# vxlerian/cpu-raymarcher

Measured on AMD Instinct MI355X. Metric: frames/sec, 3840x2160 Dense-Grid sphere-trace (+ avg SDF-calls/pixel), higher is better.
Workload: dtype f64

## Files before the change

### cpu_raymarcher_amd/_native.py

```python
import ctypes as C
import os
import subprocess

_PKG = os.path.dirname(os.path.abspath(__file__))
LIB_PATH = os.environ.get("RM_HIP_LIB") or os.path.join(_PKG, "librm_hip.so")
CSRC = os.path.join(_PKG, "csrc")

RM_OK = 0
RM_E_INVALID = -1
RM_E_UNSUPPORTED = -2
RM_E_NO_DEVICE = -3
RM_E_HIP = -4
RM_E_NO_SCENE = -5
RM_E_NOMEM = -6
RM_SCENE_UPLOADED = -(2 ** 31)

_STATUS_NAMES = {0: "RM_OK", -1: "RM_E_INVALID", -2: "RM_E_UNSUPPORTED", -3: "RM_E_NO_DEVICE",
                 -4: "RM_E_HIP", -5: "RM_E_NO_SCENE", -6: "RM_E_NOMEM"}


class RmError(RuntimeError):
    def __init__(self, code, msg):
        super().__init__("%s (%d): %s" % (_STATUS_NAMES.get(code, "?"), code, msg))
        self.code = code
# ... 137 lines not shown
    "rm_last_kernel": (C.c_char_p, [_VP]),
    "rm_version": (C.c_char_p, []),
    "rm_algorithm_from_string": (C.c_int, [C.c_char_p]),
    "rm_accel_from_string": (C.c_int, [C.c_char_p]),
    "rm_shader_from_string": (C.c_int, [C.c_char_p]),
    "rm_preset_count": (C.c_int, []),
    "rm_scene_from_preset": (C.c_int, [_VP, C.c_int32, C.c_int32]),
    "rm_scene_from_spheres": (C.c_int, [_VP, _VP, _VP, C.c_int32, C.c_int32]),
    "rm_scene_edit_spheres": (C.c_int, [_VP, C.POINTER(rm_sphere_edit), C.c_int32]),
    "rm_debug_scene_table": (C.c_int, [_VP, C.c_char_p, C.c_int32, _VP, C.c_int64, C.POINTER(C.c_int64)]),
    "rm_selftest_hypot64": (C.c_int, [_VP, _VP, C.c_int64, C.c_int32, _VP]),
    "rm_scene_from_prims": (C.c_int, [_VP, C.POINTER(rm_prim), C.c_int32, C.c_int32]),
    "rm_make_transform": (C.c_int, [C.c_double, C.c_double, C.c_double, _VP, _VP]),
    "rm_scene_from_nodes": (C.c_int, [_VP, C.POINTER(rm_node), C.c_int32, _VP, C.c_int32, C.c_int32]),
    "rm_scale_transform": (C.c_int, [_VP, C.c_double, C.c_double, C.c_double]),
    "rm_scene_set_time": (C.c_int, [_VP, C.c_double]),
    "rm_selftest_jsmath": (C.c_int, [_VP, C.c_int32, _VP, _VP, C.c_int64, _VP]),
    "rm_scene_get_info": (C.c_int, [_VP, C.POINTER(rm_scene_info)]),
    "rm_camera_from_angles": (C.c_int, [C.c_double, C.c_double, _VP, _VP]),
    "rm_scene_distance": (C.c_int, [_VP, _VP, C.c_int64, _VP, _VP]),
    "rm_debug_wave_distance": (C.c_int, [_VP, _VP, C.c_int64, _VP, _VP]),
    "rm_scene_field": (C.c_int, [_VP, C.POINTER(rm_lattice), _VP, _VP, _VP]),
    "rm_scene_field_device": (C.c_int, [_VP, C.POINTER(rm_lattice), _VP, _VP, _VP, _VP]),
    "rm_lattice_points": (C.c_int, [C.POINTER(rm_lattice), C.c_int64, C.c_int64, _VP]),
    "rm_shade_field_device": (C.c_int, [_VP, C.POINTER(rm_field_shade), C.c_int64, _VP, _VP, _VP]),
    "rm_shade_field": (C.c_int, [_VP, C.POINTER(rm_field_shade), C.c_int64, _VP, _VP]),
    "rm_mesh_field_device": (C.c_int, [_VP, C.POINTER(rm_lattice), _VP, C.c_int32, C.c_double, _VP, C.c_int64, _VP, C.c_int64, _VP, _VP]),
    "rm_scene_mesh": (C.c_int, [_VP, C.POINTER(rm_lattice), C.c_double, _VP, C.c_int64, _VP, C.c_int64, C.POINTER(rm_mesh_info)]),
    "rm_ray_march": (C.c_int, [_VP, C.POINTER(rm_ray_query), C.c_int64, _VP, _VP, _VP, _VP, _VP, _VP]),
    "rm_ray_march_device": (C.c_int, [_VP, C.POINTER(rm_ray_query), C.c_int64, _VP, _VP, _VP, _VP, _VP, _VP, _VP]),
    "rm_camera_rays": (C.c_int, [C.c_int32, C.c_int32, C.c_double, C.c_double, C.c_int32, C.c_int32, _VP, _VP]),
    "rm_ray_pick": (C.c_int, [_VP, C.POINTER(rm_ray_query), C.c_int64, _VP, _VP, _VP, _VP, _VP, _VP, _VP]),
    "rm_ray_pick_device": (C.c_int, [_VP, C.POINTER(rm_ray_query), C.c_int64, _VP, _VP, _VP, _VP, _VP, _VP, _VP, _VP]),
    "rm_ray_light": (C.c_int, [_VP, C.POINTER(rm_ray_query), C.POINTER(rm_light), C.c_int64, _VP, _VP, _VP, _VP, _VP, _VP, _VP, _VP, _VP,
                               _VP]),
    "rm_ray_light_device": (C.c_int, [_VP, C.POINTER(rm_ray_query), C.POINTER(rm_light), C.c_int64, _VP, _VP, _VP, _VP, _VP, _VP, _VP, _VP,
                                      _VP, _VP, _VP]),
    "rm_ray_walk": (C.c_int, [_VP, C.POINTER(rm_ray_query), C.c_int64, _VP, _VP, C.c_int32, _VP, _VP]),
    "rm_ray_walk_device": (C.c_int, [_VP, C.POINTER(rm_ray_query), C.c_int64, _VP, _VP, C.c_int32, _VP, _VP, _VP]),
    "rm_phong_light": (C.c_int, [_VP]),
    "rm_shade_lit_device": (C.c_int, [_VP, C.c_int32, C.c_int32, C.c_int32, _VP, _VP, _VP, _VP, _VP, _VP]),
    "rm_shade_lit": (C.c_int, [_VP, C.c_int32, C.c_int32, C.c_int32, _VP, _VP, _VP, _VP, _VP]),
    "rm_scene_object": (C.c_int, [_VP, C.c_int32, C.POINTER(rm_node), C.c_int32, C.POINTER(C.c_int32)]),
    "rm_render_tile": (C.c_int, [_VP, C.POINTER(rm_job), _VP, _VP, _VP, _VP]),
    "rm_render_tile_device": (C.c_int, [_VP, C.POINTER(rm_job), C.c_int32, _VP, _VP, _VP, _VP, _VP, _VP]),
    "rm_render_frames_device": (C.c_int, [_VP, C.POINTER(rm_job), C.c_int32, _VP, C.c_int32, _VP, _VP, _VP, _VP, _VP, _VP, _VP]),
    "rm_compare_frames_device": (C.c_int, [_VP, C.c_int32, C.c_int32, C.c_int32, C.POINTER(rm_frame_set), C.POINTER(rm_frame_set),
                                           C.c_int32, C.c_int32, _VP, _VP, _VP]),
    "rm_compare_frames": (C.c_int, [_VP, C.c_int32, C.c_int32, C.c_int32, C.POINTER(rm_frame_set), C.POINTER(rm_frame_set),
                                    C.c_int32, C.c_int32, _VP, _VP]),
    "rm_counter_hist_device": (C.c_int, [_VP, C.c_int32, C.c_int32, C.c_int32, _VP, _VP, _VP, C.c_int32, C.c_int32, C.c_int32, C.c_int32,
                                         _VP, _VP]),
    "rm_counter_hist": (C.c_int, [_VP, C.c_int32, C.c_int32, C.c_int32, _VP, _VP, _VP, C.c_int32, C.c_int32, C.c_int32, C.c_int32, _VP]),
    "rm_shade_ranged_device": (C.c_int, [_VP, C.c_int32, C.c_int32, C.c_int32, C.c_int32, _VP, _VP, C.c_uint32, C.c_uint32, _VP, _VP]),
    "rm_shade_ranged": (C.c_int, [_VP, C.c_int32, C.c_int32, C.c_int32, C.c_int32, _VP, _VP, C.c_uint32, C.c_uint32, _VP]),
    "rm_sweep_views": (C.c_int, [C.c_double, C.c_double, C.c_double, C.c_double, C.c_double, C.c_double, C.c_int32, _VP]),
    "rm_render_stripes_device": (C.c_int, [_VP, C.POINTER(rm_job), C.c_int32, C.c_int32, C.c_int32, C.c_int32,
                                           _VP, _VP, _VP, _VP, _VP, _VP]),
    "rm_stripe_rows": (C.c_int, [C.c_int32, C.c_int32, C.c_int32, C.c_int32, C.c_int32]),
    "rm_deal_stripes": (C.c_int, [C.c_int32, C.c_int32, C.c_int32, _VP, _VP]),
    "rm_render_stripe_list_device": (C.c_int, [_VP, C.POINTER(rm_job), C.c_int32, C.c_int32, _VP, C.c_int32,
                                               _VP, _VP, _VP, _VP, _VP, _VP]),
    "rm_assemble_frame_device": (C.c_int, [_VP, _VP, C.c_int64, C.c_int64, C.c_int32, C.c_int32, C.c_int32, _VP,
                                           C.c_int32, C.c_int32, _VP, C.c_int64, _VP, _VP]),
    "rm_shade": (C.c_int, [_VP, C.c_int32, C.c_int32, C.c_int32, _VP, _VP, _VP, _VP, _VP]),
    "rm_shade_device": (C.c_int, [_VP, C.c_int32, C.c_int32, C.c_int32, _VP, _VP, _VP, _VP, _VP, _VP]),
    "rm_reduce_counters": (C.c_int, [_VP, _VP, _VP, C.c_int64, C.POINTER(rm_diagnostics)]),
    "rm_reduce_counters_device": (C.c_int, [_VP, _VP, _VP, C.c_int64, C.POINTER(rm_diagnostics), _VP]),
    "rm_reduce_counters_enqueue": (C.c_int, [_VP, _VP, _VP, C.c_int64, _VP, _VP]),
    "rm_render_attach_diagnostics": (C.c_int, [_VP, _VP]),
    "rm_partition_rows": (C.c_int, [C.c_int32, C.c_int32, C.c_int32, C.POINTER(C.c_int32), C.POINTER(C.c_int32)]),
    "rm_selftest_hypot": (C.c_int, [_VP, _VP, C.c_int64, _VP]),
    "rm_selftest_fastdiv": (C.c_int, [_VP, C.c_uint64, C.c_int64, C.POINTER(C.c_uint64)]),
    "rm_selftest_recip": (C.c_int, [_VP, C.c_int, _VP]),
    "rm_debug_read_stamps": (C.c_int, [_VP, _VP]),
    "rm_debug_read_wave_times": (C.c_int, [_VP, _VP]),
    "rm_debug_read_batch_log": (C.c_int, [_VP, _VP]),
    "rm_debug_read_counts": (C.c_int, [_VP, _VP]),
    "rm_debug_read_lpt_costs": (C.c_int, [_VP, _VP, C.c_int64]),
    "rm_debug_launch_fill": (C.c_int, [_VP, C.c_int32, C.POINTER(C.c_int32)]),
    "rm_debug_last_launch": (C.c_int, [_VP, C.POINTER(C.c_uint32)]),
    "rm_debug_overlap_fill": (C.c_int, [_VP, C.c_int32, C.c_int64, C.POINTER(C.c_int32)]),
    "rm_debug_step_box": (C.c_int, [_VP, C.POINTER(C.c_int32)]),
    "rm_rtc_source": (C.c_int, [_VP, C.c_char_p, C.c_int64, C.POINTER(C.c_int64)]),
    "rm_rtc_compile_check": (C.c_int, [_VP, C.c_int32, C.c_int32, C.c_char_p, C.c_int64, C.POINTER(C.c_double)]),
    "rm_rtc_status": (C.c_int, [_VP, C.POINTER(C.c_int32), C.POINTER(C.c_int32), C.c_char_p, C.c_int64]),
    "rm_set_option": (C.c_int, [_VP, C.c_char_p, C.c_int64]),
    "rm_get_option": (C.c_int, [_VP, C.c_char_p, C.POINTER(C.c_int64)]),
}

_lib = None


def build(force=False, verbose=False):
    srcs = [os.path.join(CSRC, f) for f in os.listdir(CSRC) if f.endswith((".hip", ".cpp", ".h"))]
    srcs.append(os.path.join(os.path.dirname(_PKG), "include", "rm_raymarch.h"))
    if not force and os.path.exists(LIB_PATH) and all(
            os.path.getmtime(LIB_PATH) >= os.path.getmtime(s) for s in srcs):
        return LIB_PATH
    cmd = ["make", "-j%d" % min(8, os.cpu_count() or 1), "-C", CSRC, "all"] + (["-B"] if force else [])
    subprocess.check_call(cmd, stdout=None if verbose else subprocess.DEVNULL)
    return LIB_PATH


def lib():
    global _lib
    if _lib is None:
        if not os.path.exists(LIB_PATH):
            raise ImportError(
                "cpu_raymarcher_amd: %s is missing. Build it with `python -c 'import __graft_entry__ as g; "
                "g.build()'` or `make -C cpu_raymarcher_amd/csrc`. There is no CPU fallback." % LIB_PATH)
        try:
            import torch
        except ImportError:
            pass
        L = C.CDLL(LIB_PATH)
        for name, (res, args) in SIGNATURES.items():
            if os.environ.get("RM_HIP_LIB") and not hasattr(L, name):
                continue
            fn = getattr(L, name)
            fn.restype = res
            fn.argtypes = args
        _lib = L
    return _lib


def check(ctx, rc):
    if rc == RM_OK:
        return
    msg = lib().rm_last_error(ctx).decode() if ctx else ""
    raise (RmUnsupported if rc == RM_E_UNSUPPORTED else RmError)(rc, msg)
```

### cpu_raymarcher_amd/context.py

```python
import ctypes as C

import numpy as np

from . import _native as N


def _is_torch(x):
    return type(x).__module__.startswith("torch")


def _ptr(x):
    if x is None:
        return None
    if _is_torch(x):
        return C.c_void_p(x.data_ptr())
    return x.ctypes.data_as(C.c_void_p)


_BPP = {"depth": 1, "normal": 3, "sdf": 2, "iters": 2, "rgba": 4}


def _check_buffers(npx, bufs, need_device=None):
    on_dev = None
    for name, b in bufs.items():
# ... 50 lines not shown
    if not (_is_torch(hist) or isinstance(hist, np.ndarray)):
        raise ValueError("hist must be a numpy array or a torch tensor")
    d = bool(_is_torch(hist) and hist.is_cuda)
    contiguous = hist.is_contiguous() if _is_torch(hist) else hist.flags["C_CONTIGUOUS"]
    nbytes = hist.numel() * hist.element_size() if _is_torch(hist) else hist.nbytes
    if not contiguous or nbytes < 2128 * max(0, n_frames):
        raise ValueError("hist must be a contiguous buffer of 2128 bytes per frame")
    if on_dev is not None and on_dev != d:
        raise ValueError("buffers must be all on the host or all on the device")
    return d


def percentile(record, permille):
    p = int(permille)
    if not 0 <= p <= 1000:
        raise ValueError("permille must be in [0, 1000]")
    M = int(record["pixels"])
    if M == 0:
        return 0, 0
    r = p * (M - 1) // 1000
    b = int(np.searchsorted(np.cumsum(np.asarray(record["bins"], dtype=np.uint64)), r, side="right"))
    shift, mn, mx = int(record["shift"]), int(record["min"]), int(record["max"])
    return max(mn, b << shift), (mx if b == 255 else min(mx, ((b + 1) << shift) - 1))


def _current_stream_ptr():
    import torch
    return C.c_void_p(torch.cuda.current_stream().cuda_stream)


class Context:

    def __init__(self, device=0):
        self._h = C.c_void_p()
        self.device = -1 if device is None else int(device)
        rc = N.lib().rm_create(self.device, C.byref(self._h))
        if rc != N.RM_OK:
            raise N.RmError(rc, "rm_create(device=%d) failed: no usable HIP device" % self.device)

    def close(self):
        if self._h:
            N.lib().rm_destroy(self._h)
            self._h = C.c_void_p()

    def __del__(self):
        try:
            self.close()
        except Exception:
            pass

    def __enter__(self):
        return self

    def __exit__(self, *a):
        self.close()

    def set_option(self, key, value):
        N.check(self._h, N.lib().rm_set_option(self._h, key.encode(), int(value)))

    def get_option(self, key):
        v = C.c_int64(0)
        N.check(self._h, N.lib().rm_get_option(self._h, key.encode(), C.byref(v)))
        return v.value

    def launch_fill(self, asked):
        v = C.c_int32(0)
        N.check(self._h, N.lib().rm_debug_launch_fill(self._h, int(asked), C.byref(v)))
        return v.value

    def last_launch(self):
        out = (C.c_uint32 * 4)()
        N.check(self._h, N.lib().rm_debug_last_launch(self._h, out))
        return dict(workgroups=out[0], threads=out[1], lds_bytes=out[2], cus=out[3])

    def overlap_fill(self, asked, items):
        v = C.c_int32(0)
        N.check(self._h, N.lib().rm_debug_overlap_fill(self._h, int(asked), int(items), C.byref(v)))
        return v.value

    def step_box(self):
        out = (C.c_int32 * 6)()
        N.check(self._h, N.lib().rm_debug_step_box(self._h, out))
        return dict(last=bool(out[0]), planned=bool(out[1]), reason=out[2], list_cap=out[3], list_cap_without=out[4], table_bytes=out[5])

    def scene_from_preset(self, index, accel):
        N.check(self._h, N.lib().rm_scene_from_preset(self._h, int(index), int(accel)))

    def scene_from_spheres(self, centers, radii, accel):
        c = np.ascontiguousarray(centers, dtype=np.float32).reshape(-1, 3)
        r = np.ascontiguousarray(radii, dtype=np.float64).reshape(-1)
        if len(c) != len(r):
            raise ValueError("centers and radii differ in length")
        N.check(self._h, N.lib().rm_scene_from_spheres(self._h, _ptr(c), _ptr(r), len(r), int(accel)))

    def scene_from_prims(self, prims, accel):
        prims = list(prims)
        arr = (N.rm_prim * max(1, len(prims)))()
        for i, (t, m, par) in enumerate(prims):
            arr[i].type = int(t)
            for k in range(16):
                arr[i].world_to_local[k] = float(m[k])
            for k in range(3):
                arr[i].params[k] = float(par[k]) if k < len(par) else 0.0
        N.check(self._h, N.lib().rm_scene_from_prims(self._h, arr, len(prims), int(accel)))

    def scene_from_nodes(self, nodes, roots, accel):
        nodes = list(nodes)
        arr = (N.rm_node * max(1, len(nodes)))()
        for i, (t, a, b, m, par) in enumerate(nodes):
            arr[i].type, arr[i].child_a, arr[i].child_b = int(t), int(a), int(b)
            for k in range(16):
                arr[i].world_to_local[k] = 0.0 if m is None else float(m[k])
            for k in range(6):
                arr[i].params[k] = float(par[k]) if k < len(par) else 0.0
        r = np.ascontiguousarray(roots, dtype=np.int32)
        N.check(self._h, N.lib().rm_scene_from_nodes(self._h, arr, len(nodes), _ptr(r), len(r), int(accel)))

    def edit_spheres(self, edits):
        if isinstance(edits, C.Array) and edits._type_ is N.rm_sphere_edit:
            arr, n = edits, len(edits)
        else:
            edits = list(edits)
            n = len(edits)
            arr = (N.rm_sphere_edit * max(1, n))()
            for k, e in enumerate(edits):
                arr[k].op = N.EDIT_OPS[e[0]] if isinstance(e[0], str) else int(e[0])
                arr[k].index = int(e[1])
                if len(e) > 2:
                    arr[k].center[:] = [float(v) for v in np.asarray(e[2], np.float32).reshape(3)]
                    arr[k].radius = float(e[3])
        N.check(self._h, N.lib().rm_scene_edit_spheres(self._h, arr, n))

    def scene_table(self, name, from_device=True):
        size = C.c_int64(0)
        key = name.encode()
        N.check(self._h, N.lib().rm_debug_scene_table(self._h, key, int(bool(from_device)), None, 0, C.byref(size)))
        out = np.zeros(size.value, np.uint8)
        N.check(self._h, N.lib().rm_debug_scene_table(self._h, key, int(bool(from_device)), _ptr(out), out.size, C.byref(size)))
        return out.view(N.SCENE_TABLES.get(name, "u1"))

    def selftest_hypot64(self, xyz, on_device=True):
        a = np.ascontiguousarray(xyz, dtype=np.float64).reshape(-1, 3)
        out = np.zeros(len(a), np.float64)
        N.check(self._h, N.lib().rm_selftest_hypot64(self._h, _ptr(a), len(a), int(bool(on_device)), _ptr(out)))
        return out

    def scene_set_time(self, time):
        N.check(self._h, N.lib().rm_scene_set_time(self._h, float(time)))

    def selftest_jsmath(self, fn, a, b=None):
        a = np.ascontiguousarray(a, dtype=np.float64)
        b = None if b is None else np.ascontiguousarray(b, dtype=np.float64)
        out = np.zeros_like(a)
        N.check(self._h, N.lib().rm_selftest_jsmath(self._h, int(fn), _ptr(a), _ptr(b), a.size, _ptr(out)))
        return out

    def scene_info(self):
        info = N.rm_scene_info()
        N.check(self._h, N.lib().rm_scene_get_info(self._h, C.byref(info)))
        d = {k: getattr(info, k) for k, _ in info._fields_ if k not in ("root_min", "root_max", "reserved")}
        d["root_min"] = [float(v) for v in info.root_min]
        d["root_max"] = [float(v) for v in info.root_max]
        d["prog_slots"], d["prog_vals"], d["prog_instructions"] = info.program & 0xFF, (info.program >> 8) & 0xFF, info.program >> 16
        return d

    def scene_distance(self, points):
# ... 710 lines not shown
```

### cpu_raymarcher_amd/csrc/rm_api.cpp

```cpp
#include <hip/hip_runtime_api.h>

#include <algorithm>
#include <array>
#include <cerrno>
#include <climits>
#include <cmath>
#include <cstdio>
#include <cstdlib>
#include <cstring>
#include <functional>
#include <limits>
#include <map>
#include <unordered_map>
#include <new>
#include <string>
#include <vector>

#include "../../include/rm_raymarch.h"
#include "rm_diag.h"
#include "rm_kernels.h"
#include "rm_rtc.h"
#include "rm_scene_host.h"

namespace {

#define RM_SCENE_ARRAYS(X)                                                                                                        \
    X(spheres, 1) X(radii, 1) X(bvh, 1) X(bvh_prims, 1) X(oct, 1) X(oct_prims, 1) X(pq_cells, 1) X(pq_list, 1) X(nn_cells, 1)      \
    X(nn_list, 1) X(prims, 1) X(prog, 1) X(obj_ranges, 1) X(oct_recs, 1) X(oct_lut, 1) X(oct_sub_hdr, 1) X(oct_sub_list, 1)       \
    X(slot_object, 0) X(ext_cells, 1) X(ext_list, 1) X(step_tab, 1)

struct DeviceScene {
#define RM_X(name, always) decltype(rmh::HostScene::name)::value_type *name = nullptr;
    RM_SCENE_ARRAYS(RM_X)
#undef RM_X
    uint16_t *bvh_leaves = nullptr;
    int32_t bvh_leaf_count = 0;
};

struct SceneDesc {
    enum Kind { kSpheres, kPrims, kNodes } kind = kSpheres;
    std::vector<float> centers;
    std::vector<double> radii;
    std::vector<rmh::PrimDesc> prims;
    std::vector<rmh::NodeDesc> nodes;
    std::vector<int> roots;
};

struct LaunchSlots {
    static constexpr unsigned kLaunches = 1024, kHeads = 64, kHeadWords = 64;
    unsigned int *heads = nullptr;
    RmDiagBlock *blocks = nullptr;
    unsigned int head_slot = 0, block_slot = 0;

    hipError_t init() {
        const size_t head_bytes = sizeof(unsigned int) * kLaunches * kHeads * kHeadWords, block_bytes = sizeof(RmDiagBlock) * kLaunches;
        hipError_t e = hipMalloc(reinterpret_cast<void **>(&heads), head_bytes);
        if (e == hipSuccess) e = hipMemset(heads, 0, head_bytes);
        if (e == hipSuccess) e = hipMalloc(reinterpret_cast<void **>(&blocks), block_bytes);
        return e == hipSuccess ? hipMemset(blocks, 0, block_bytes) : e;
    }
    void release() {
        (void)hipFree(heads);
        (void)hipFree(blocks);
    }
    unsigned int *take_heads() { return heads ? heads + static_cast<size_t>(kHeads) * kHeadWords * (head_slot++ % kLaunches) : nullptr; }
    RmDiagBlock *take_block() { return blocks ? blocks + block_slot++ % kLaunches : nullptr; }
};

struct RingClaims {
    struct Claim {
        size_t first, n;
        hipEvent_t done;
    };
    size_t next = 0;
    std::vector<Claim> claims;

    void retire_all() {
        for (Claim &c : claims) (void)hipEventDestroy(c.done);
        claims.clear();
        next = 0;
    }
    hipError_t take(size_t n, size_t cap, size_t *first) {
        if (next + n > cap) next = 0;
        const size_t lo = next, hi = next + n;
        for (size_t k = 0; k < claims.size();) {
            const Claim c = claims[k];
            if (c.first < hi && lo < c.first + c.n) {
                const hipError_t e = hipEventSynchronize(c.done);
                if (e != hipSuccess) return e;
                (void)hipEventDestroy(c.done);
                claims.erase(claims.begin() + static_cast<std::ptrdiff_t>(k));
            } else ++k;
        }
        *first = lo;
        next = hi;
        return hipSuccess;
    }
    void launched(size_t first, size_t n, hipStream_t stream) {
        hipEvent_t ev = nullptr;
        if (hipEventCreateWithFlags(&ev, hipEventDisableTiming) == hipSuccess && hipEventRecord(ev, stream) == hipSuccess) {
            claims.push_back(Claim{first, n, ev});
            return;
        }
        if (ev) (void)hipEventDestroy(ev);
        (void)hipStreamSynchronize(stream);
    }
};

struct FrameRing {
    static constexpr size_t kFrames = 4096;
    RmFrameView *host = nullptr, *dev = nullptr;
    RmFrameDiagBlock *blocks = nullptr;
    size_t cap = 0;
    RingClaims owners;

    void release() {
        owners.retire_all();
        (void)hipHostFree(host);
        (void)hipFree(dev);
        (void)hipFree(blocks);
        host = dev = nullptr;
        blocks = nullptr;
        cap = 0;
    }
    hipError_t take(size_t n, size_t *first) {
        if (n > cap) {
            hipError_t e = hipDeviceSynchronize();
            if (e != hipSuccess) return e;
            release();
            const size_t want = n > kFrames ? n : kFrames;
            e = hipHostMalloc(reinterpret_cast<void **>(&host), want * sizeof(RmFrameView), hipHostMallocDefault);
            if (e == hipSuccess) e = hipMalloc(reinterpret_cast<void **>(&dev), want * sizeof(RmFrameView));
            if (e == hipSuccess) e = hipMalloc(reinterpret_cast<void **>(&blocks), want * sizeof(RmFrameDiagBlock));
            if (e == hipSuccess) e = hipMemset(blocks, 0, want * sizeof(RmFrameDiagBlock));
            if (e != hipSuccess) {
                release();
                return e;
            }
            cap = want;
        }
        return owners.take(n, cap, first);
    }
    void launched(size_t first, size_t n, hipStream_t stream) { owners.launched(first, n, stream); }
};

struct CompareRing {
    static constexpr size_t kEntries = 4096;
// ... 133 lines not shown
        for (auto &u : t.users) {
            (void)hipEventSynchronize(u.second);
            (void)hipEventDestroy(u.second);
        }
        t.users.clear();
        t.valid = false;
        const size_t n = static_cast<size_t>(oct_nodes);
        if (t.nodes < n) {
            (void)hipFree(t.dev);
            t.dev = nullptr;
            t.nodes = 0;
            if (hipMalloc(reinterpret_cast<void **>(&t.dev), n * sizeof(RmOctFrameNode)) == hipSuccess) t.nodes = n;
            else (void)hipGetLastError();
        }
        if (!t.dev || rm_launch_oct_frame_table(oct, oct_nodes, origin, t.dev, stream) != hipSuccess) return nullptr;
        for (int a = 0; a < 3; ++a) t.origin[a] = origin[a];
        t.gen = gen;
        t.valid = true;
        t.builder = stream;
        if (!t.built && hipEventCreateWithFlags(&t.built, hipEventDisableTiming) != hipSuccess) t.built = nullptr;
        if (!t.built || hipEventRecord(t.built, stream) != hipSuccess) (void)hipStreamSynchronize(stream);
        cur = k;
        return &t;
    }
    static void read_by(Table &t, hipStream_t stream) {
        hipEvent_t ev = nullptr;
        for (auto &u : t.users)
            if (u.first == stream) ev = u.second;
        if (!ev) {
            if (hipEventCreateWithFlags(&ev, hipEventDisableTiming) == hipSuccess) t.users.emplace_back(stream, ev);
            else ev = nullptr;
        }
        if (ev) (void)hipEventRecord(ev, stream);
        else (void)hipStreamSynchronize(stream);
    }
    void release() {
        for (Table &t : slots) {
            (void)hipFree(t.dev);
            for (auto &u : t.users) (void)hipEventDestroy(u.second);
            if (t.built) (void)hipEventDestroy(t.built);
        }
    }
};

}

struct rm_ctx {
    int device = -1;
    bool has_device = false;
    std::string err = "";
    hipStream_t stream = nullptr;

    bool have_scene = false;
    bool scene_is_uploaded = false;
    int scene_preset = 0;
    rmh::HostScene host;
    DeviceScene dev;

    bool have_uploaded = false;
    SceneDesc uploaded;
    double time = 0.0;

    void *scratch = nullptr;
    size_t scratch_bytes = 0;
    hipEvent_t scratch_busy = nullptr;
    RmDiagDevice *d_diag = nullptr;
    float light[3] = {0, 0, 0};

    int64_t opt_tile_w = 8;
    bool tile_w_set = false;
    int64_t opt_filter = 1;
    int64_t opt_lds = 1;
    int64_t opt_kernel = 0;
    int64_t opt_list_cap = 32;
    int64_t opt_coop = 1;
    int64_t opt_grid = 1;
    int64_t opt_nn = 2;
    int64_t opt_ext = 1;
    int64_t opt_blocks_per_cu = 6;
    int64_t opt_lds_fill = 0;
    int64_t opt_min_fill = 1;
    int64_t opt_overlap_fill = 1;
    int hw_queues = 4;
    uint32_t last_v2_shape[4] = {0, 0, 0, 0};
    int64_t opt_item_wide = 0;
    int64_t opt_multi_step = 1;
    int64_t opt_step_box = 1;
    int64_t opt_lds_kb = 0;
    int64_t opt_refill = 64;
    int64_t opt_recs = 1;
    int64_t opt_static = 0;
    int64_t opt_lut = 1;
    int64_t opt_cull = 1;
    int64_t opt_rel = 1;
    int64_t opt_uniform = 1;
    int64_t opt_sub = 1;
    int64_t opt_hw_xcd = 1;
    int64_t opt_v1_lists = 1;
    int64_t opt_v1_block = 64;
    int64_t opt_oct_lean = 1;
    int64_t opt_lpt = 1;
    LaunchSlots slots;
    LptRing lpt;
    OctTableRing oct_tables;
    FrameRing frames;
    CompareRing compare;
    HistRing hists;
    unsigned long long scene_gen = 0;
    int64_t opt_n0_batch = 64;
    int64_t opt_length = 0;
    const char *last_kernel = "";
    std::string last_kernel_kept;
    int64_t opt_device_build = 1;
    int64_t opt_specialise = 1;
    int64_t opt_rtc_spheres = 16;
    int64_t opt_prune = 1;
    std::string rtc_src;
    std::map<int, rmrtc::Kernel> rtc_kernels;
    std::vector<rmrtc::Kernel> rtc_owned;
    std::map<int, std::string> rtc_failed;
    std::string rtc_log;
    struct V2Special {
        int launches = 0;
        int state = 0;
        bool lite = false;
        rmrtc::Kernel k;
    };
    std::unordered_map<uint64_t, V2Special> v2_special;
    int64_t opt_v2_after = 3;
    struct DevTable {
        std::vector<int32_t> host;
        int32_t *dev = nullptr;
    };
    std::vector<DevTable> tables;
    int64_t opt_item_px = 128;
    void *diag_next = nullptr;
    unsigned long long *d_stamps = nullptr;
    int num_cus = 256;
};

namespace {

int fail(rm_ctx *ctx, int code, const std::string &msg) {
    if (ctx) ctx->err = msg;
    return code;
}

int hip_fail(rm_ctx *ctx, hipError_t e, const char *what) {
    return fail(ctx, RM_E_HIP, std::string(what) + ": " + hipGetErrorString(e));
}

int read_hw_queues() {
    const char *s = std::getenv("GPU_MAX_HW_QUEUES");
    if (!s || !*s) return 4;
    char *end = nullptr;
    errno = 0;
    const long long v = std::strtoll(s, &end, 10);
    if (errno || end == s || *end != '\0' || v <= 0) return 4;
    return static_cast<int>(std::min<long long>(v, INT_MAX));
}

int launch_fill(int asked, int queues, bool min_fill) {
    if (!min_fill) return asked;
    const int q = queues > 0 ? queues : 4;
    return std::max(asked, (RM_V2_WAVES + q - 1) / q);
}

int overlap_fill(int asked, int queues, bool min_fill, bool overlap) {
    const int floor = launch_fill(asked, queues, min_fill);
    const int q = queues > 0 ? queues : 4;
    if (!min_fill || !overlap || q >= RM_V2_WAVES) return floor;
    const int per_mille = 436 * q;
    return std::max(floor, std::min(RM_V2_WAVES, (RM_V2_WAVES * 1000 + per_mille - 1) / per_mille));
}

int obtain_kernel(rm_ctx *ctx, const std::string &src, int accel, bool other, bool length_sqrt, rmrtc::Kernel &k) {
    if (ctx->opt_specialise == 2) return rmrtc::compile_async(ctx->device, src, accel, other, length_sqrt, k, ctx->rtc_log);
    bool cached = false;
    if (!rmrtc::compile_cached(ctx->device, src, accel, other, length_sqrt, k, ctx->rtc_log, &cached)) return -1;
    if (!cached) ctx->rtc_owned.push_back(k);
    return 1;
}

const rmrtc::Kernel *specialised_kernel(rm_ctx *ctx, int accel, bool other) {
    if (!ctx->opt_specialise || ctx->rtc_src.empty() || !ctx->has_device) return nullptr;
    const int key = (accel * 2 + (other ? 1 : 0)) * 2 + (ctx->opt_length ? 1 : 0);
    auto it = ctx->rtc_kernels.find(key);
    if (it != ctx->rtc_kernels.end()) return &it->second;
    if (ctx->rtc_failed.count(key)) return nullptr;
    rmrtc::Kernel k;
    const int st = obtain_kernel(ctx, ctx->rtc_src, accel, other, ctx->opt_length != 0, k);
    if (st < 0) ctx->rtc_failed[key] = ctx->rtc_log;
    if (st <= 0) return nullptr;
    return &(ctx->rtc_kernels[key] = k);
}

}

const void *rm_rtc_v2_hook(const RmRenderParams &p, int accel, bool lds, bool ur, bool rel, bool length_sqrt) {
    rm_ctx *ctx = static_cast<rm_ctx *>(p.rtc_ctx);
    if (!ctx || !ctx->opt_specialise || ctx->opt_v2_after <= 0) return nullptr;
    const int bits = (accel & 3) | (lds ? 4 : 0) | (ur ? 8 : 0) | (rel ? 16 : 0) | rmrtc::kV2Bit;
    rm_ctx::V2Special &e = ctx->v2_special[rmrtc::v2_fixed_hash(p, bits | (length_sqrt ? 512 : 0))];
    if (e.state == 1) return e.k.render;
    if (e.state < 0) return nullptr;
    if (e.state == 0 && ++e.launches < ctx->opt_v2_after) return nullptr;
    for (;;) {
        const int st = obtain_kernel(ctx, rmrtc::v2_fixed_source(p, !e.lite), bits, false, length_sqrt, e.k);
        e.state = st > 0 ? 1 : (st < 0 ? -1 : 2);
        if (st >= 0 || e.lite) break;
        e.lite = true;
        e.state = 0;
    }
    return e.state == 1 ? e.k.render : nullptr;
}

namespace {

hipError_t launch_render(rm_ctx *ctx, const RmRenderParams &p_in, RmDiagDevice *diag_out, hipStream_t stream) {
    RmRenderParams p = p_in;
#if !defined(RM_STAMPS) && !defined(RM_COUNTS) && !defined(RM_STAMPS_LOG) && !defined(RM_STAMPS_CLAIM)
    p.rtc_ctx = ctx;
#endif
    const bool empty = p.local_rows <= 0 || p.width <= 0;
    const bool v2 = p.variant == 2 && p.algorithm == 0;
    const bool lean_oct = p.accel == 1 && p.oct_lean && !p.general && p.algorithm == 0 && p.oct_lut && p.oct_recs && p.filter;
    const rmrtc::Kernel *special = v2 || lean_oct ? nullptr : specialised_kernel(ctx, p.accel, p.algorithm != 0);
    p.rtc_function = special ? special->render : nullptr;
    OctTableRing::Table *oct_table = lean_oct ? ctx->oct_tables.acquire(ctx->scene_gen, p.oct, p.oct_nodes, p.origin_d, stream) : nullptr;
    p.oct_frame = oct_table ? oct_table->dev : nullptr;
    if (ctx->opt_lpt && v2) ctx->lpt.acquire(p);
    if (v2 && !empty) p.tile_counters = ctx->slots.take_heads();
    p.diag_out = diag_out;
    RmDiagDevice *reduce_after = nullptr;
    if (p.diag_out && !v2 && !empty && p.sdf && p.iters) {
        reduce_after = p.diag_out;
        p.diag_out = nullptr;
    }
    p.diag_block = !empty && (p.diag_out || v2) ? ctx->slots.take_block() : nullptr;
    if (p.diag_out && empty) {
        const hipError_t ei = rm_launch_reduce_init(p.diag_out, stream);
        if (ei != hipSuccess) return ei;
    }
    hipError_t e = ctx->opt_length ? rm_launch_render_sqrt(p, stream, &ctx->last_kernel, ctx->last_v2_shape)
                                   : rm_launch_render(p, stream, &ctx->last_kernel, ctx->last_v2_shape);
    if (special && !empty) ctx->last_kernel = special->name.c_str();
    if (e == hipSuccess && reduce_after) {
        e = rm_launch_reduce_init(reduce_after, stream);
        if (e == hipSuccess) e = rm_launch_reduce(p.sdf, p.iters, static_cast<int64_t>(p.local_rows) * p.width, reduce_after, stream);
    }
    if (oct_table) OctTableRing::read_by(*oct_table, stream);
    if (e == hipSuccess && p.lpt_perm_out) ctx->lpt.launched(stream);
    return e;
}

#define RM_HIP(ctx, call)                                       \
    do {                                                        \
        hipError_t e_ = (call);                                 \
        if (e_ != hipSuccess) return hip_fail(ctx, e_, #call); \
    } while (0)

#define RM_NEED_DEVICE(ctx, text)                                             \
    do {                                                                      \
        if (!(ctx)) return RM_E_INVALID;                                      \
        if (!(ctx)->has_device) return fail(ctx, RM_E_NO_DEVICE, text);       \
    } while (0)

void free_device_scene(rm_ctx *ctx) {
    for (auto &k : ctx->rtc_owned) rmrtc::release(k);
    ctx->rtc_owned.clear();
    ctx->rtc_kernels.clear();
    ctx->v2_special.clear();
    ctx->rtc_failed.clear();
    ctx->last_kernel = "";
    if (!ctx->has_device) return;
    DeviceScene &d = ctx->dev;
#define RM_X(name, always) (void)hipFree(d.name);
    RM_SCENE_ARRAYS(RM_X)
#undef RM_X
    (void)hipFree(d.bvh_leaves);
    d = DeviceScene();
}

int device_table(rm_ctx *ctx, const int32_t *host, size_t n, const int32_t **out) {
    for (auto &t : ctx->tables)
        if (t.host.size() == n && std::memcmp(t.host.data(), host, n * sizeof(int32_t)) == 0) {
            *out = t.dev;
            return RM_OK;
        }
    if (ctx->tables.size() >= 256) {
        RM_HIP(ctx, hipDeviceSynchronize());
        for (auto &t : ctx->tables) (void)hipFree(t.dev);
        ctx->tables.clear();
    }
    rm_ctx::DevTable t;
    t.host.assign(host, host + n);
    RM_HIP(ctx, hipMalloc(reinterpret_cast<void **>(&t.dev), (n ? n : 1) * sizeof(int32_t)));
    if (n) RM_HIP(ctx, hipMemcpy(t.dev, host, n * sizeof(int32_t), hipMemcpyHostToDevice));
    *out = t.dev;
    ctx->tables.push_back(std::move(t));
    return RM_OK;
}

template <typename T>
int upload_vec(rm_ctx *ctx, const std::vector<T> &v, T **out) {
    *out = nullptr;
    const size_t bytes = (v.empty() ? 1 : v.size()) * sizeof(T);
    RM_HIP(ctx, hipMalloc(reinterpret_cast<void **>(out), bytes));
    if (!v.empty()) RM_HIP(ctx, hipMemcpy(*out, v.data(), v.size() * sizeof(T), hipMemcpyHostToDevice));
    return RM_OK;
}

std::vector<uint16_t> cull_leaf_table(const std::vector<RmBvhNode> &bvh) {
    std::vector<uint16_t> leaves;
    bool ok = !bvh.empty() && bvh.size() < 65536;
    std::vector<int> parent(bvh.size(), -1);
    for (size_t i = 0; ok && i < bvh.size(); ++i) {
        if (bvh[i].leaf >= 0) continue;
        for (size_t c = i + 1; c < static_cast<size_t>(bvh[i].skip) && c < bvh.size(); c = static_cast<size_t>(bvh[c].skip)) {
            parent[c] = static_cast<int>(i);
            if (bvh[c].skip <= static_cast<int>(c)) { ok = false; break; }
        }
    }
    for (size_t i = 0; ok && i < bvh.size(); ++i) {
        if (parent[i] >= 0)
            for (int k = 0; k < 3; ++k)
                if (!(bvh[i].lo[k] >= bvh[parent[i]].lo[k] && bvh[i].hi[k] <= bvh[parent[i]].hi[k])) ok = false;
        for (int k = 0; k < 3; ++k)
            if (!(bvh[i].lo[k] <= bvh[i].hi[k])) ok = false;
        if (i > 0 && parent[i] < 0) ok = false;
        if (bvh[i].leaf >= 0 && (bvh[i].leaf & 0xFF) > 0) leaves.push_back(static_cast<uint16_t>(i));
    }
    if (!ok || leaves.size() > 256) leaves.clear();
    return leaves;
}

int upload_scene(rm_ctx *ctx) {
    ctx->rtc_src.clear();
    if (ctx->host.program) {
        ctx->rtc_src = rmrtc::scene_source(ctx->host.prog, ctx->host.obj_ranges, ctx->host.prog_tree, ctx->host.prog_roots, ctx->opt_prune != 0, ctx->host.bvh,
                                           ctx->host.bvh_prims, false);
    } else if (ctx->host.general ? ctx->host.prims.size() <= 32 : static_cast<int64_t>(ctx->host.spheres.size()) < ctx->opt_rtc_spheres) {
        std::vector<RmInstr> prog;
        std::vector<int32_t> ranges, roots;
        std::vector<rmh::ProgTreeNode> tree;
        if (rmh::leaf_objects(ctx->host, prog, ranges, tree, roots))
            ctx->rtc_src = rmrtc::scene_source(prog, ranges, tree, roots, false, ctx->host.bvh, ctx->host.bvh_prims, true);
    }
    if (!ctx->has_device) {
        free_device_scene(ctx);
        return RM_OK;
    }
    RM_HIP(ctx, hipSetDevice(ctx->device));
    RM_HIP(ctx, hipDeviceSynchronize());
    free_device_scene(ctx);
    ctx->scene_gen++;
    int rc;
#define RM_X(name, always) \
    if ((always || !ctx->host.name.empty()) && (rc = upload_vec(ctx, ctx->host.name, &ctx->dev.name))) return rc;
    RM_SCENE_ARRAYS(RM_X)
#undef RM_X
    const std::vector<uint16_t> leaves = cull_leaf_table(ctx->host.bvh);
    ctx->dev.bvh_leaf_count = static_cast<int32_t>(leaves.size());
    return upload_vec(ctx, leaves, &ctx->dev.bvh_leaves);
}

int clamp_preset(int idx) { return idx < 0 ? 0 : (idx > rmh::kPresetCount - 1 ? rmh::kPresetCount - 1 : idx); }
int norm_accel(int a) { return (a == RM_ACCEL_OCTREE || a == RM_ACCEL_BVH) ? a : RM_ACCEL_NONE; }

int set_scene(rm_ctx *ctx, const SceneDesc &d, int accel, bool uploaded, int preset, const rmh::PairLoops *loops = nullptr) {
    std::string err;
    rmh::HostScene hs;
    rmh::set_length_mode(static_cast<int>(ctx->opt_length));
    bool ok = false;
    switch (d.kind) {
        case SceneDesc::kSpheres: ok = rmh::build_scene(hs, d.centers.data(), d.radii.data(), static_cast<int>(d.radii.size()), accel, err, loops); break;
        case SceneDesc::kPrims: ok = rmh::build_scene_general(hs, d.prims.data(), static_cast<int>(d.prims.size()), accel, err); break;
        case SceneDesc::kNodes:
            ok = rmh::build_scene_nodes(hs, d.nodes.data(), static_cast<int>(d.nodes.size()), d.roots.data(), static_cast<int>(d.roots.size()), accel, err);
            break;
    }
    if (!ok) {
        const bool unsupported = err.find("BVH leaf") != std::string::npos || (d.kind == SceneDesc::kNodes && err.find("RM_PROG_MAX") != std::string::npos);
        return fail(ctx, unsupported ? RM_E_UNSUPPORTED : RM_E_INVALID, err);
    }
    hs.preset = preset;
    ctx->host = std::move(hs);
    ctx->have_scene = true;
    ctx->scene_is_uploaded = uploaded;
    ctx->scene_preset = preset;
    return upload_scene(ctx);
}

int set_uploaded_scene(rm_ctx *ctx, SceneDesc &&d, int32_t accel) {
    const int rc = set_scene(ctx, d, norm_accel(accel), true, RM_SCENE_UPLOADED);
    if (rc) return rc;
    ctx->uploaded = std::move(d);
    ctx->have_uploaded = true;
    return RM_OK;
}

bool preset_desc(int preset, SceneDesc &d) {
    d.kind = SceneDesc::kSpheres;
    if (rmh::preset_spheres(preset, d.centers, d.radii)) return true;
    d.kind = SceneDesc::kPrims;
    if (rmh::preset_prims(preset, d.prims)) return true;
    d.kind = SceneDesc::kNodes;
    return rmh::preset_nodes(preset, d.nodes, d.roots);
}


struct DevMem {
    void *p = nullptr;
    DevMem() = default;
    DevMem(const DevMem &) = delete;
    DevMem &operator=(const DevMem &) = delete;
    ~DevMem() {
        if (p) (void)hipFree(p);
    }
    hipError_t alloc(size_t bytes) { return hipMalloc(&p, bytes ? bytes : 1); }
    template <typename T>
    hipError_t put(const T *src, size_t n, hipStream_t stream) {
        hipError_t e = alloc(n * sizeof(T));
        if (e == hipSuccess && n) e = hipMemcpyAsync(p, src, n * sizeof(T), hipMemcpyHostToDevice, stream);
        return e;
    }
    template <typename T>
    T *as() const { return static_cast<T *>(p); }
};

#define RM_TRY(call)                            \
    do {                                        \
        if ((call) != hipSuccess) return false; \
    } while (0)

template <typename E>
bool device_cand_lists(rm_ctx *ctx, const rmh::HostScene &s, const std::vector<int32_t> *ids, const std::vector<RmCandGrid> &grids,
                       int cells_per_grid, double u0, bool use_root, bool cap255, const std::vector<uint32_t> *order,
                       std::vector<uint32_t> &hdr, std::vector<E> &list) {
    const size_t n = s.spheres.size(), n_cells = grids.size() * static_cast<size_t>(cells_per_grid);
    if (!n || !n_cells || n != s.radii.size() || n > 0x7FFFFFFFu || (order && order->size() != n_cells)) return false;
    RM_TRY(hipSetDevice(ctx->device));
    hipStream_t st = ctx->stream;
    std::vector<double> sp(4 * n);
    for (size_t i = 0; i < n; ++i) {
        sp[4 * i] = s.spheres[i].cx;
        sp[4 * i + 1] = s.spheres[i].cy;
// ... 177 lines not shown
        for (const RmInstr &ins : ctx->host.prog)
            if (ins.op == 3) p.general = 3;
    }
    p.prims = ctx->dev.prims;
    p.prog = ctx->dev.prog;
    p.obj_ranges = ctx->dev.obj_ranges;
    p.prog_slots = ctx->host.prog_slots;
    p.prog_vals = ctx->host.prog_vals;
    p.accel = ctx->host.accel;
    p.bvh_nodes = static_cast<int32_t>(ctx->host.bvh.size());
    p.oct_nodes = static_cast<int32_t>(ctx->host.oct.size());
    p.spheres = ctx->dev.spheres;
    p.radii = ctx->dev.radii;
    p.bvh = ctx->dev.bvh;
    p.bvh_prims = ctx->dev.bvh_prims;
    p.oct = ctx->dev.oct;
    p.oct_prims = ctx->dev.oct_prims;
    p.oct_lut = ctx->opt_lut ? ctx->dev.oct_lut : nullptr;
    p.ext_cells = ctx->dev.ext_cells;
    p.ext_list = ctx->dev.ext_list;
    for (int k = 0; k < 3; ++k) {
        p.ext_dim[k] = ctx->host.ext_dim[k];
        p.ext_origin[k] = ctx->host.ext_origin[k];
        p.ext_inv[k] = ctx->host.ext_inv[k];
    }
    p.use_ext = (ctx->opt_ext && ctx->host.accel == RM_ACCEL_BVH && !ctx->host.ext_cells.empty() && ctx->host.ext_dim[0] > 0) ? 1 : 0;
}


int ensure_scene(rm_ctx *ctx, int32_t preset_index, int32_t accel_in) {
    const int accel = norm_accel(accel_in);
    if (preset_index == RM_SCENE_UPLOADED) {
        if (!ctx->have_uploaded) return fail(ctx, RM_E_NO_SCENE, "no scene uploaded with rm_scene_from_spheres");
        if (ctx->have_scene && ctx->scene_is_uploaded && ctx->host.accel == accel) return RM_OK;
        return set_scene(ctx, ctx->uploaded, accel, true, RM_SCENE_UPLOADED);
    }
    const int preset = clamp_preset(preset_index);
    if (ctx->have_scene && !ctx->scene_is_uploaded && ctx->scene_preset == preset && ctx->host.accel == accel)
        return RM_OK;
    SceneDesc d;
    if (preset_desc(preset, d)) return set_scene(ctx, d, accel, false, preset);
    return fail(ctx, RM_E_UNSUPPORTED, "scene preset " + std::to_string(preset) + " is not on the native path");
}

size_t align_up(size_t v, size_t a) { return (v + a - 1) / a * a; }

struct Staging {
    rm_ctx *ctx;
    size_t total = 0;
    size_t region(size_t bytes) {
        const size_t offset = total;
        total += align_up(bytes, 256);
        return offset;
    }
    int reserve() const { return reserve_for(ctx->stream); }
    int reserve_for(hipStream_t user) const {
        if (ctx->scratch_busy) RM_HIP(ctx, hipStreamWaitEvent(user, ctx->scratch_busy, 0));
        const size_t bytes = total ? total : 256;
        if (bytes <= ctx->scratch_bytes) return RM_OK;
        if (ctx->scratch) {
            RM_HIP(ctx, hipDeviceSynchronize());
            (void)hipFree(ctx->scratch);
            ctx->scratch = nullptr;
            ctx->scratch_bytes = 0;
        }
        RM_HIP(ctx, hipMalloc(&ctx->scratch, bytes));
        ctx->scratch_bytes = bytes;
        return RM_OK;
    }
    template <typename T>
    T *at(size_t offset) const { return reinterpret_cast<T *>(static_cast<char *>(ctx->scratch) + offset); }
    hipError_t in(size_t offset, const void *host, size_t bytes) const { return hipMemcpyAsync(at<char>(offset), host, bytes, hipMemcpyHostToDevice, ctx->stream); }
    hipError_t zero(size_t offset, size_t bytes) const { return hipMemsetAsync(at<char>(offset), 0, bytes, ctx->stream); }
    hipError_t out(void *host, size_t offset, size_t bytes) const { return hipMemcpyAsync(host, at<char>(offset), bytes, hipMemcpyDeviceToHost, ctx->stream); }
    hipError_t sync() const { return hipStreamSynchronize(ctx->stream); }
    hipError_t keep(hipStream_t user) const {
        if (!ctx->scratch_busy) {
            const hipError_t e = hipEventCreateWithFlags(&ctx->scratch_busy, hipEventDisableTiming);
            if (e != hipSuccess) return e;
        }
        return hipEventRecord(ctx->scratch_busy, user);
    }
};

int fill_params(rm_ctx *ctx, const rm_job *job, RmRenderParams &p) {
    if (!job) return fail(ctx, RM_E_INVALID, "null job");
    if (job->height <= 0 || job->width < 0) return fail(ctx, RM_E_INVALID, "width must be >= 0 and height > 0");
    if (!std::isfinite(job->camera_pitch) || !std::isfinite(job->camera_yaw))
        return fail(ctx, RM_E_INVALID, "non-finite camera angle");
    if (job->algorithm < RM_ALG_SPHERE_TRACER || job->algorithm > RM_ALG_ADAPTIVE_STEP_V3)
        return fail(ctx, RM_E_INVALID, "unknown algorithm enum (use rm_algorithm_from_string)");
    int rc = ensure_scene(ctx, job->scene_preset_index, job->acceleration_structure);
    if (rc) return rc;
    std::memset(&p, 0, sizeof p);
    p.width = job->width;
    p.height = job->height;
    p.y_start = job->y_start;
    p.y_end = job->y_end;
    p.algorithm = job->algorithm;
    p.overshoot = std::isnan(job->overshoot_factor) ? 1.2 : job->overshoot_factor;
    p.step_size = std::isnan(job->step_size) ? 0.1 : job->step_size;
    p.local_rows = job->y_end > job->y_start ? job->y_end - job->y_start : 0;
    p.stripe_rows = 0;
    p.n_parts = 1;
    p.part = 0;
    rmh::camera_from_angles(job->camera_pitch, job->camera_yaw, p.rot, p.origin);
    std::memcpy(p.light, ctx->light, sizeof p.light);
    for (int k = 0; k < 9; ++k) p.rot_d[k] = p.rot[k];
    for (int k = 0; k < 3; ++k) {
        p.origin_d[k] = p.origin[k];
        p.light_d[k] = p.light[k];
    }
    fill_scene_view(ctx, p);
    if (!std::isfinite(job->time)) return fail(ctx, RM_E_INVALID, "non-finite time");
    ctx->time = job->time;
    p.time = job->time;
    p.tile_w = static_cast<int32_t>(ctx->opt_tile_w);
    p.nodes_in_lds = static_cast<int32_t>(ctx->opt_lds);
    p.filter = static_cast<int32_t>(ctx->opt_filter);
    p.variant = static_cast<int32_t>(ctx->opt_kernel);
    if (p.variant == 0)
        p.variant = (ctx->host.accel == RM_ACCEL_OCTREE || ctx->host.spheres.size() < 8 ||
                     (ctx->opt_specialise && !ctx->rtc_src.empty() && rmrtc::available(nullptr) &&
                      static_cast<int64_t>(ctx->host.spheres.size()) < ctx->opt_rtc_spheres))
                        ? 1
                        : 2;
    if (p.algorithm != RM_ALG_SPHERE_TRACER) p.variant = 1;
    if (ctx->host.general) p.variant = 1;
    if (p.variant == 1 && !ctx->tile_w_set) p.tile_w = 8;
    p.list_cap = static_cast<int32_t>(ctx->opt_list_cap);
    p.coop = static_cast<int32_t>(ctx->opt_coop);
    p.bvh_prim_count = static_cast<int32_t>(ctx->host.bvh_prims.size());
    p.oct_prim_count = static_cast<int32_t>(ctx->host.oct_prims.size());
    p.blocks_per_cu = static_cast<int32_t>(ctx->opt_blocks_per_cu);
    p.launch_per_cu = launch_fill(p.blocks_per_cu, ctx->hw_queues, ctx->opt_min_fill != 0);
    p.overlap_per_cu = overlap_fill(p.blocks_per_cu, ctx->hw_queues, ctx->opt_min_fill != 0, ctx->opt_overlap_fill != 0);
    p.num_cus = ctx->num_cus;
    p.refill_threshold = static_cast<int32_t>(ctx->opt_refill);
    p.hw_xcd = static_cast<int32_t>(ctx->opt_hw_xcd);
    p.item_px = static_cast<int32_t>(ctx->opt_item_px);
    p.stamps = ctx->d_stamps;
    for (int k = 0; k < 3; ++k) {
        p.pq_dim[k] = ctx->host.pq_dim[k];
        p.pq_origin[k] = ctx->host.pq_origin[k];
        p.pq_inv[k] = ctx->host.pq_inv[k];
        p.pq_cell[k] = ctx->host.pq_inv[k] > 0.f ? static_cast<float>((1.0 / static_cast<double>(ctx->host.pq_inv[k])) * 0.9999) : 0.f;
    }
    p.pq_cell_count = static_cast<int32_t>(ctx->host.pq_cells.size());
    p.pq_list_count = static_cast<int32_t>(ctx->host.pq_list.size());
    p.use_grid = (ctx->opt_grid && !ctx->host.pq_cells.empty()) ? 1 : 0;
    p.pq_cells = ctx->dev.pq_cells;
    p.pq_list = ctx->dev.pq_list;
    p.bvh_leaves = ctx->dev.bvh_leaves;
    p.bvh_leaf_count = (ctx->opt_cull && ctx->host.accel == RM_ACCEL_BVH) ? ctx->dev.bvh_leaf_count : 0;
    p.nn_cells = ctx->dev.nn_cells;
    p.nn_list = ctx->dev.nn_list;
    p.nn_cell_count = static_cast<int32_t>(ctx->host.nn_cells.size());
    p.nn_list_count = static_cast<int32_t>(ctx->host.nn_list.size());
    const bool nn_on = ctx->opt_nn == 1 || (ctx->opt_nn == 2 && ctx->host.spheres.size() <= 512);
    p.use_nn = (p.use_grid && nn_on && !ctx->host.nn_cells.empty()) ? 1 : 0;
    p.leaf_order = ctx->host.leaf_order ? 1 : 0;
    p.rel_boxes = static_cast<int32_t>(ctx->opt_rel);
    p.n0_batch = static_cast<int32_t>(ctx->opt_n0_batch);
    p.v1_lists = static_cast<int32_t>(ctx->opt_v1_lists);
    p.v1_block = static_cast<int32_t>(ctx->opt_v1_block);
    p.oct_lean = static_cast<int32_t>(ctx->opt_oct_lean);
    p.v1_list_offset = -1;
    p.prim_filter = (ctx->opt_filter && ctx->host.general && !ctx->host.program && ctx->host.prim_filter_ok &&
                     ctx->host.spheres.size() == ctx->host.prims.size()) ? 1 : 0;
    p.lds_budget_kb = static_cast<int32_t>(ctx->opt_lds_kb);
    p.lds_fill = static_cast<int32_t>(ctx->opt_lds_fill);
    p.item_wide = static_cast<int32_t>(ctx->opt_item_wide);
    p.multi_step = static_cast<int32_t>(ctx->opt_multi_step);
    p.step_tab = ctx->dev.step_tab;
    p.sb_bins = ctx->host.sb_bins;
    p.sb_stride = ctx->host.sb_stride;
    for (int k = 0; k < 3; ++k) {
        p.sb_origin[k] = ctx->host.sb_origin[k];
        p.sb_inv[k] = ctx->host.sb_inv[k];
    }
    p.step_box = (ctx->opt_step_box && ctx->opt_multi_step && ctx->host.accel == RM_ACCEL_BVH && !ctx->host.step_tab.empty() &&
                  (ctx->dev.step_tab || !ctx->has_device)) ? 1 : 0;
    p.uniform_radius = 0;
    if (ctx->opt_uniform && !ctx->host.general && ctx->host.spheres.size() >= 2 &&
        ctx->host.spheres.size() <= 256) {
        const auto &sp = ctx->host.spheres;
        const auto &rd = ctx->host.radii;
        bool same = rd.size() == sp.size();
        for (size_t k = 1; same && k < sp.size(); ++k)
            same = std::memcmp(&sp[k].rf, &sp[0].rf, sizeof(float)) == 0 && std::memcmp(&rd[k], &rd[0], sizeof(double)) == 0;
        p.uniform_radius = same ? 1 : 0;
    }
    for (int k = 0; k < 3; ++k) {
        p.nn_dim[k] = ctx->host.nn_dim[k];
        p.nn_inv[k] = ctx->host.nn_inv[k];
    }
    p.oct_recs = ctx->opt_recs ? ctx->dev.oct_recs : nullptr;
    p.oct_sub_hdr = (ctx->opt_sub && ctx->opt_recs) ? ctx->dev.oct_sub_hdr : nullptr;
    p.oct_sub_list = ctx->dev.oct_sub_list;
    return RM_OK;
}

template <typename Launch>
int read_mismatches(rm_ctx *ctx, Launch launch, uint64_t *mismatches) {
    RM_HIP(ctx, hipSetDevice(ctx->device));
    Staging st{ctx};
    const size_t o = st.region(sizeof(unsigned long long));
    const int rc = st.reserve();
    if (rc) return rc;
    RM_HIP(ctx, st.zero(o, sizeof(unsigned long long)));
    RM_HIP(ctx, launch(st.at<unsigned long long>(o)));
    unsigned long long h = 0;
    RM_HIP(ctx, st.out(&h, o, sizeof h));
    RM_HIP(ctx, st.sync());
    *mismatches = h;
    return RM_OK;
}

int norm_shader(int s) { return (s >= RM_SHADE_NORMAL && s <= RM_SHADE_ITERATION_HEATMAP) ? s : RM_SHADE_NORMAL; }

int fill_query_params(rm_ctx *ctx, const rm_ray_query *q, RmRenderParams &p) {
    const double scene_time = ctx->time;
    rm_job job;
    std::memset(&job, 0, sizeof job);
    job.width = 1;
    job.height = 1;
    job.y_end = 1;
    job.time = q->time;
    const bool known = q->algorithm >= RM_ALG_SPHERE_TRACER && q->algorithm <= RM_ALG_ADAPTIVE_STEP_V3;
    job.algorithm = known ? q->algorithm : RM_ALG_SPHERE_TRACER;
    job.scene_preset_index = ctx->scene_is_uploaded ? RM_SCENE_UPLOADED : ctx->scene_preset;
    job.acceleration_structure = ctx->host.accel;
    job.overshoot_factor = q->overshoot_factor;
    job.step_size = q->step_size;
    const int rc = fill_params(ctx, &job, p);
    ctx->time = scene_time;
    p.rtc_function = nullptr;
// ... 1680 lines not shown
    const bool ok = rmrtc::compile(ctx->rtc_src, norm_accel(accel), other != 0, ctx->opt_length != 0, false, k, text);
    if (seconds) *seconds = k.compile_seconds;
    copy_text(text, log, cap, nullptr);
    if (ok) return RM_OK;
    if (text.compare(0, 8, "refused:") == 0) return fail(ctx, RM_E_UNSUPPORTED, "hiprtc: the specialised kernel spills and would not be loaded (see the log)");
    return fail(ctx, RM_E_INVALID, "hiprtc: the specialised kernel did not compile (see the log)");
}

int rm_rtc_status(rm_ctx *ctx, int32_t *compiled, int32_t *failed, char *log, int64_t cap) {
    if (!ctx) return RM_E_INVALID;
    int v2_ready = 0, v2_failed = 0;
    for (const auto &kv : ctx->v2_special) {
        v2_ready += kv.second.state == 1;
        v2_failed += kv.second.state < 0;
    }
    if (compiled) *compiled = static_cast<int32_t>(ctx->rtc_kernels.size()) + v2_ready;
    if (failed) *failed = static_cast<int32_t>(ctx->rtc_failed.size()) + v2_failed;
    std::string why;
    if (!rmrtc::available(&why)) return copy_text(why, log, cap, nullptr);
    return copy_text(ctx->rtc_log, log, cap, nullptr);
}

int rm_debug_read_lpt_costs(rm_ctx *ctx, uint8_t *out, int64_t n) {
    if (!out) return RM_E_INVALID;
    RM_NEED_DEVICE(ctx, "host-only context");
    const uint8_t *costs = ctx->lpt.last_costs();
    if (!costs || n < 0 || static_cast<size_t>(n) > LptRing::kPerSlot) return fail(ctx, RM_E_INVALID, "no costs recorded");
    RM_HIP(ctx, hipSetDevice(ctx->device));
    RM_HIP(ctx, hipDeviceSynchronize());
    RM_HIP(ctx, hipMemcpy(out, costs, static_cast<size_t>(n), hipMemcpyDeviceToHost));
    return RM_OK;
}

int rm_debug_launch_fill(rm_ctx *ctx, int32_t asked, int32_t *effective) {
    if (!ctx || !effective) return RM_E_INVALID;
    if (asked < 1 || asked > 8) return fail(ctx, RM_E_INVALID, "blocks_per_cu must be in [1, 8]");
    *effective = launch_fill(asked, ctx->hw_queues, ctx->opt_min_fill != 0);
    return RM_OK;
}

int rm_debug_overlap_fill(rm_ctx *ctx, int32_t asked, int64_t items, int32_t *effective) {
    if (!ctx || !effective) return RM_E_INVALID;
    if (asked < 1 || asked > 8) return fail(ctx, RM_E_INVALID, "blocks_per_cu must be in [1, 8]");
    if (items < 0) return fail(ctx, RM_E_INVALID, "items must not be negative");
    const bool min_fill = ctx->opt_min_fill != 0;
    *effective = rm_v2_overlap_per_cu(launch_fill(asked, ctx->hw_queues, min_fill),
                                      overlap_fill(asked, ctx->hw_queues, min_fill, ctx->opt_overlap_fill != 0), items, ctx->num_cus);
    return RM_OK;
}

int rm_debug_last_launch(rm_ctx *ctx, uint32_t out[4]) {
    if (!ctx || !out) return RM_E_INVALID;
    for (int k = 0; k < 3; ++k) out[k] = ctx->last_v2_shape[k];
    out[3] = static_cast<uint32_t>(ctx->num_cus);
    return RM_OK;
}

int rm_debug_step_box(rm_ctx *ctx, int32_t out[6]) {
    if (!ctx || !out) return RM_E_INVALID;
    for (int k = 0; k < 6; ++k) out[k] = 0;
    out[0] = static_cast<int32_t>(ctx->last_v2_shape[3]);
    if (!ctx->have_scene) return fail(ctx, RM_E_NO_SCENE, "no scene set");
    rm_job job;
    std::memset(&job, 0, sizeof job);
    job.width = job.height = job.y_end = 64;
    job.algorithm = RM_ALG_SPHERE_TRACER;
    job.scene_preset_index = ctx->scene_is_uploaded ? RM_SCENE_UPLOADED : ctx->scene_preset;
    job.acceleration_structure = ctx->host.accel;
    job.overshoot_factor = job.step_size = std::nan("");
    const double scene_time = ctx->time;
    RmRenderParams p;
    const int rc = fill_params(ctx, &job, p);
    ctx->time = scene_time;
    if (rc) return rc;
    out[5] = static_cast<int32_t>(ctx->host.step_tab.size() * sizeof(uint32_t));
    RmRenderParams plain = p;
    plain.step_box = 0;
    out[4] = rm_v2_plan(plain).list_cap;
    const RmV2Plan plan = rm_v2_plan(p);
    out[3] = plan.list_cap;
    const bool v2 = p.variant == 2 && p.algorithm == 0 && p.accel == 2;
    out[1] = v2 && plan.step_box ? 1 : 0;
    out[2] = out[1] ? 0 : (ctx->host.step_tab.empty() && v2 && ctx->opt_step_box && ctx->opt_multi_step ? 2 : (v2 && plan.refused ? 3 : 1));
    return RM_OK;
}

enum OptionKind {
    kSwitch,
    kRange,
    kZeroOrRange,
    kSet,
};
struct OptionRow {
    const char *key;
    int64_t rm_ctx::*member;
    OptionKind kind;
    int64_t v[4];
    const char *error;
};
static const OptionRow kOptions[] = {
    {"tile_w", &rm_ctx::opt_tile_w, kSet, {8, 16, 32, 64}, "tile_w must be 8, 16, 32 or 64"},
    {"filter", &rm_ctx::opt_filter, kSwitch, {}, nullptr},
    {"nodes_in_lds", &rm_ctx::opt_lds, kSwitch, {}, nullptr},
    {"kernel", &rm_ctx::opt_kernel, kRange, {0, 2}, "kernel must be 0 (auto), 1 or 2"},
    {"list_cap", &rm_ctx::opt_list_cap, kRange, {1, 64}, "list_cap must be in [1, 64]"},
    {"coop", &rm_ctx::opt_coop, kSwitch, {}, nullptr},
    {"recs", &rm_ctx::opt_recs, kSwitch, {}, nullptr},
    {"lut", &rm_ctx::opt_lut, kSwitch, {}, nullptr},
    {"uniform", &rm_ctx::opt_uniform, kSwitch, {}, nullptr},
    {"lds_kb", &rm_ctx::opt_lds_kb, kZeroOrRange, {16, 64}, "lds_kb must be 0 (auto) or in [16, 64]"},
    {"multi_step", &rm_ctx::opt_multi_step, kSwitch, {}, nullptr},
    {"step_box", &rm_ctx::opt_step_box, kSwitch, {}, nullptr},
    {"item_wide", &rm_ctx::opt_item_wide, kSwitch, {}, nullptr},
    {"prune", &rm_ctx::opt_prune, kSwitch, {}, nullptr},
    {"rtc_spheres", &rm_ctx::opt_rtc_spheres, kRange, {0, 33}, "rtc_spheres must be 0..33"},
    {"specialise_v2_after", &rm_ctx::opt_v2_after, kRange, {0, 1000000}, "specialise_v2_after must be 0 (never) .. 1000000 launches"},
    {"specialise", &rm_ctx::opt_specialise, kRange, {0, 2}, "specialise must be 0, 1 or 2"},
    {"lds_fill", &rm_ctx::opt_lds_fill, kSwitch, {}, nullptr},
    {"min_fill", &rm_ctx::opt_min_fill, kSwitch, {}, nullptr},
    {"overlap_fill", &rm_ctx::opt_overlap_fill, kSwitch, {}, nullptr},
    {"cull", &rm_ctx::opt_cull, kSwitch, {}, nullptr},
    {"rel", &rm_ctx::opt_rel, kSwitch, {}, nullptr},
    {"static", &rm_ctx::opt_static, kRange, {0, 95}, "static must be in [0, 95] percent"},
    {"sub", &rm_ctx::opt_sub, kSwitch, {}, nullptr},
    {"refill", &rm_ctx::opt_refill, kRange, {1, 64}, "refill must be in [1, 64]"},
    {"item_px", &rm_ctx::opt_item_px, kSet, {64, 128, 256, 256}, "item_px must be 64, 128 or 256"},
    {"hw_xcd", &rm_ctx::opt_hw_xcd, kSwitch, {}, nullptr},
    {"grid", &rm_ctx::opt_grid, kSwitch, {}, nullptr},
    {"nn", &rm_ctx::opt_nn, kRange, {0, 2}, "nn must be 0 (off), 1 (on) or 2 (auto)"},
    {"ext", &rm_ctx::opt_ext, kSwitch, {}, nullptr},
    {"blocks_per_cu", &rm_ctx::opt_blocks_per_cu, kRange, {1, 8}, "blocks_per_cu must be in [1, 8]"},
    {"v1_lists", &rm_ctx::opt_v1_lists, kSwitch, {}, nullptr},
    {"v1_block", &rm_ctx::opt_v1_block, kSet, {64, 128, 256, 256}, "v1_block must be 64, 128 or 256"},
    {"oct_lean", &rm_ctx::opt_oct_lean, kSwitch, {}, nullptr},
    {"lpt", &rm_ctx::opt_lpt, kSwitch, {}, nullptr},
    {"n0_batch", &rm_ctx::opt_n0_batch, kRange, {1, 64}, "n0_batch must be in [1, 64]"},
    {"device_build", &rm_ctx::opt_device_build, kSwitch, {}, nullptr},
    {"length", &rm_ctx::opt_length, kRange, {0, 1}, "length must be 0 (Math.hypot) or 1 (Math.sqrt)"},
};

static const OptionRow *find_option(const char *key) {
    for (const OptionRow &o : kOptions)
        if (!std::strcmp(key, o.key)) return &o;
    return nullptr;
}

int rm_set_option(rm_ctx *ctx, const char *key, int64_t value) {
    if (!ctx || !key) return RM_E_INVALID;
    const OptionRow *o = find_option(key);
    if (!o) return fail(ctx, RM_E_INVALID, std::string("unknown option ") + key);
    bool ok = true;
    switch (o->kind) {
        case kSwitch: value = value ? 1 : 0; break;
        case kRange: ok = value >= o->v[0] && value <= o->v[1]; break;
        case kZeroOrRange: ok = value == 0 || (value >= o->v[0] && value <= o->v[1]); break;
        case kSet: ok = std::find(std::begin(o->v), std::end(o->v), value) != std::end(o->v); break;
    }
    if (!ok) return fail(ctx, RM_E_INVALID, o->error);
    const bool changed = ctx->*(o->member) != value;
    ctx->*(o->member) = value;
    if (o->member == &rm_ctx::opt_tile_w) ctx->tile_w_set = true;
    if (o->member == &rm_ctx::opt_length && changed && ctx->have_scene) {
        ctx->have_scene = false;
        return ensure_scene(ctx, ctx->scene_is_uploaded ? RM_SCENE_UPLOADED : ctx->scene_preset, ctx->host.accel);
    }
    return RM_OK;
}

int rm_get_option(const rm_ctx *ctx, const char *key, int64_t *value) {
    if (!ctx || !key || !value) return RM_E_INVALID;
    const OptionRow *o = find_option(key);
    if (!o) return RM_E_INVALID;
    *value = ctx->*(o->member);
    return RM_OK;
}

}
```

### cpu_raymarcher_amd/csrc/rm_kernels.h

```cpp
#pragma once
#ifndef __HIPCC_RTC__
#include <hip/hip_runtime_api.h>
#include <stdint.h>
#endif

#include "rm_types.h"

struct RmDiagDevice {
    unsigned long long total_sdf;
    unsigned long long total_iters;
    unsigned int max_sdf;
    unsigned int min_sdf;
    unsigned long long pad;
};

#ifdef RM_LENGTH_SQRT
#define RM_LEN_VARIANT(name) name##_sqrt
#define RM_LEN_TAG " [length=sqrt]"
#define RM_LEN_IS_SQRT true
#else
#define RM_LEN_VARIANT(name) name
#define RM_LEN_TAG ""
#define RM_LEN_IS_SQRT false
#endif

enum { RM_CMP_NONE = -1, RM_CMP_SDF = 0, RM_CMP_ITERS = 1, RM_CMP_DEPTH = 2, RM_CMP_NORMAL = 3, RM_CMP_SURFACE = 4 };
struct RmCompareStats {
    unsigned long long pixels;
    unsigned long long sums[14];
    unsigned int max_abs_depth, max_abs_normal;
};
struct RmComparePartial {
    unsigned long long v[16];
};
struct RmCompareArgs {
    const uint8_t *depth_a, *depth_b, *normal_a, *normal_b;
    const uint16_t *sdf_a, *sdf_b, *iters_a, *iters_b;
    uint8_t *rgba;
    RmCompareStats *stats;
    RmComparePartial *partials;
    unsigned int *counters;
    long long npx;
    unsigned int gain;
};

constexpr int RM_HIST_NBINS = 256;
struct RmCounterHist {
    unsigned long long pixels, sum;
    unsigned int min, max, range_lo, range_hi, shift, reserved;
    unsigned int bins[RM_HIST_NBINS];
};
struct RmFrameHist {
    RmCounterHist sdf, iters;
};
struct RmHistScratch {
    unsigned int bins[2][RM_HIST_NBINS];
    unsigned long long sum[2];
    unsigned int max[2], inv_min[2];
    unsigned int ticket, pad[3];
};
struct RmHistArgs {
    const uint16_t *sdf, *iters;
    const uint8_t *normal;
    RmFrameHist *hist;
    RmHistScratch *scratch;
    long long npx;
    unsigned int shift, lo_permille, hi_permille;
    unsigned int want_surface;
};
struct RmShadeRangedArgs {
    const uint16_t *values;
    const RmFrameHist *hist;
    uint8_t *rgba;
    long long npx;
    unsigned int counter, lo, hi;
};
struct RmShadeLitArgs {
    const uint8_t *depth, *normal;
    const float *lit, *ao;
    uint8_t *rgba;
    long long npx;
    double light[3];
};
struct RmRays {
    const float *origins, *dirs;
    long long n;
};
struct RmQueryArgs {
    int32_t want_normal, pad;
    const int32_t *slot_obj;
    double *t;
    uint32_t *iters, *sdf;
    float *normal;
    int32_t *object;
};
struct RmLightArgs {
    const float *origins, *dirs;
    double *t;
    uint32_t *iters, *sdf;
    float *normal;
    float *lit, *ao;
    uint32_t *iters2, *sdf2;
    long long n;
    double bias, ao_step, ao_strength;
    float light[3];
    int ao_samples;
};
// ... 16 lines not shown
};
struct RmFieldArgs {
    double origin[3], du[3], dv[3], dw[3];
    double *dist;
    float *dist32;
    uint32_t *count;
    long long first, n;
    long long block_first;
    unsigned int nu, nv;
};
struct RmShadeFieldArgs {
    const void *values;
    uint8_t *rgba;
    long long n;
    double range, band, line;
    unsigned int lo, hi;
    int map, pad;
};
#define RM_MESH_BLOCK 256
#define RM_MESH_SCAN_STEP 1024
struct RmMeshInfo {
    long long n_vertices, n_quads, n_holes, reserved;
};
struct RmMeshArgs {
    double origin[3], du[3], dv[3], dw[3];
    const void *values;
    double iso;
    float *vertices;
    uint32_t *quads;
    RmMeshInfo *info;
    uint32_t *map;
    uint32_t *totals;
    long long n, cap_vertices, cap_quads;
    unsigned int nu, nv, nw, n_blocks;
    int f32, pad;
};
struct RmCandGrid {
    double org[3], w[3];
    int32_t dim[3];
    int32_t first, n, pad;
};
#define RM_CAND_NO_LIST 0xFFFFFFFFu
struct RmCandArgs {
    const RmCandGrid *grids;
    const double *spheres;
    const int32_t *ids;
    uint32_t *counts;
    double *u;
    const uint32_t *offsets;
    long long n_cells;
    unsigned long long list_len;
    double u0;
    double root_lo[3], root_hi[3];
    int32_t n_grids, cells_per_grid, n_spheres, n_ids, use_root, pad;
};
struct RmEmptyDistArgs {
    const float *boxes, *prim_lo, *prim_hi;
    double *out;
    int32_t n_nodes, n_prims;
};

#ifndef __HIPCC_RTC__
hipError_t rm_launch_cand_count(const RmCandArgs &a, hipStream_t stream);
hipError_t rm_launch_cand_fill(const RmCandArgs &a, void *list, int elem_bytes, hipStream_t stream);
hipError_t rm_launch_empty_dist(const RmEmptyDistArgs &a, hipStream_t stream);
hipError_t rm_launch_hypot64(const double *xyz, int64_t n, double *out, hipStream_t stream);

hipError_t rm_launch_render(const RmRenderParams &p, hipStream_t stream, const char **kernel_name, uint32_t *v2_shape = nullptr);
hipError_t rm_launch_render_sqrt(const RmRenderParams &p, hipStream_t stream, const char **kernel_name, uint32_t *v2_shape = nullptr);

const void *rm_rtc_v2_hook(const RmRenderParams &p, int accel, bool lds, bool ur, bool rel, bool length_sqrt);

hipError_t rm_launch_render_v2(const RmRenderParams &p, hipStream_t stream, const char **kernel_name, uint32_t *shape = nullptr);
hipError_t rm_launch_render_v2_sqrt(const RmRenderParams &p, hipStream_t stream, const char **kernel_name, uint32_t *shape = nullptr);

#define RM_V2_OVERLAP_ITEMS_PER_WAVE 3
inline int rm_v2_overlap_per_cu(int floor_per_cu, int candidate, long long items, int cus) {
    if (candidate <= floor_per_cu || cus <= 0) return floor_per_cu;
    const long long needed = (items + 3) / 4, resident = static_cast<long long>(cus) * candidate;
    const long long waves = 4 * (needed < resident ? needed : resident);
    return items >= RM_V2_OVERLAP_ITEMS_PER_WAVE * waves ? candidate : floor_per_cu;
}

struct RmV2Plan {
    bool lds, rel;
    int list_cap, step_box, tier, refused;
    size_t scene_bytes, list_bytes;
};
RmV2Plan rm_v2_plan(const RmRenderParams &p);

hipError_t rm_launch_wave_distance(const RmRenderParams &p, const float *points, int64_t n, double *dist, uint32_t *count, hipStream_t stream);
hipError_t rm_launch_wave_distance_sqrt(const RmRenderParams &p, const float *points, int64_t n, double *dist, uint32_t *count, hipStream_t stream);

hipError_t rm_launch_oct_frame_table(const RmOctNode *nodes, int n, const double origin[3], RmOctFrameNode *out, hipStream_t stream);

hipError_t rm_launch_shade(int shader, int64_t n, const uint8_t *depth, const uint8_t *normal,
                           const uint16_t *sdf, const uint16_t *iters, uint8_t *rgba,
                           const float light[3], hipStream_t stream);

hipError_t rm_launch_reduce_init(RmDiagDevice *acc, hipStream_t stream);

hipError_t rm_launch_reduce(const uint16_t *sdf, const uint16_t *iters, int64_t n, RmDiagDevice *acc,
                            hipStream_t stream);

hipError_t rm_launch_distance(const RmRenderParams &p, const float *points, int64_t n, double *dist,
                              uint32_t *count, hipStream_t stream);
hipError_t rm_launch_distance_sqrt(const RmRenderParams &p, const float *points, int64_t n, double *dist,
                                   uint32_t *count, hipStream_t stream);

hipError_t rm_launch_cast(const RmRenderParams &p, const RmRays &r, const RmQueryArgs &a, hipStream_t stream, const char **kernel_name);
hipError_t rm_launch_cast_sqrt(const RmRenderParams &p, const RmRays &r, const RmQueryArgs &a, hipStream_t stream, const char **kernel_name);
hipError_t rm_launch_pick(const RmRenderParams &p, const RmRays &r, const RmQueryArgs &a, hipStream_t stream, const char **kernel_name);
hipError_t rm_launch_pick_sqrt(const RmRenderParams &p, const RmRays &r, const RmQueryArgs &a, hipStream_t stream, const char **kernel_name);
hipError_t rm_launch_light(const RmRenderParams &p, const RmRays &r, const RmLightArgs &a, hipStream_t stream, const char **kernel_name);
hipError_t rm_launch_light_sqrt(const RmRenderParams &p, const RmRays &r, const RmLightArgs &a, hipStream_t stream, const char **kernel_name);
hipError_t rm_launch_walk(const RmRenderParams &p, const RmRays &r, const RmWalkArgs &a, hipStream_t stream, const char **kernel_name);
hipError_t rm_launch_walk_sqrt(const RmRenderParams &p, const RmRays &r, const RmWalkArgs &a, hipStream_t stream, const char **kernel_name);

hipError_t rm_launch_field(const RmRenderParams &p, const RmFieldArgs &a, hipStream_t stream, const char **kernel_name);
hipError_t rm_launch_field_sqrt(const RmRenderParams &p, const RmFieldArgs &a, hipStream_t stream, const char **kernel_name);

hipError_t rm_launch_mesh(const RmMeshArgs &a, hipStream_t stream, const char **kernel_name);

hipError_t rm_launch_frames(const RmRenderParams &p, const RmFrameView *views, int32_t n_views, RmFrameDiagBlock *blocks, RmDiagDevice *acc,
                            hipStream_t stream, const char **kernel_name);
hipError_t rm_launch_frames_sqrt(const RmRenderParams &p, const RmFrameView *views, int32_t n_views, RmFrameDiagBlock *blocks, RmDiagDevice *acc,
                                 hipStream_t stream, const char **kernel_name);

hipError_t rm_launch_lpt_sort(const uint8_t *cost_prev, uint16_t *perm, int stride, int tiles_x, int tiles_y, hipStream_t stream);

hipError_t rm_launch_assemble(const unsigned char *gathered, int64_t rank_stride, int64_t section_offset, int32_t row_bytes,
                              int32_t height, int32_t stripe_rows, const int32_t *stripe_src, int32_t n_stripes,
                              unsigned char *frame, int64_t acc_offset, int32_t world, RmDiagDevice *acc, hipStream_t stream);

int32_t rm_compare_blocks_per_frame(int64_t npx, int32_t n_frames);
hipError_t rm_launch_compare(const RmCompareArgs &a, int32_t map, int32_t n_frames, int32_t blocks_per_frame, hipStream_t stream,
                             const char **kernel_name);

hipError_t rm_launch_hist(const RmHistArgs &a, bool masked, int32_t n_frames, int32_t blocks_per_frame, hipStream_t stream,
                          const char **kernel_name);
hipError_t rm_launch_shade_ranged(const RmShadeRangedArgs &a, int32_t n_frames, hipStream_t stream, const char **kernel_name);
hipError_t rm_launch_shade_lit(const RmShadeLitArgs &a, int32_t n_frames, hipStream_t stream, const char **kernel_name);
hipError_t rm_launch_shade_field(const RmShadeFieldArgs &a, hipStream_t stream, const char **kernel_name);

hipError_t rm_launch_hypot(const float *xyz, int64_t n, double *out, hipStream_t stream);
hipError_t rm_launch_jsmath(int fn, const double *a, const double *b, int64_t n, double *out, hipStream_t stream);

hipError_t rm_launch_fastdiv_selftest(uint64_t seed, int64_t n, unsigned long long *d_mismatches, hipStream_t stream);
hipError_t rm_launch_recip_selftest(int mode, unsigned long long *d_mismatches, hipStream_t stream);
#endif
```

### cpu_raymarcher_amd/csrc/rm_render_v2.hip

```cpp
#ifndef __HIPCC_RTC__
#include <hip/hip_runtime.h>
#endif

#include "rm_device.h"
#ifdef RM_RTC_V2
#include "rm_v2_fixed.inc"
#endif

#ifdef RM_COUNTS
__shared__ unsigned int rm_cnt_s[32];
#define RM_CNT(i)                                                                                  \
    {                                                                                              \
        const unsigned int n_ = static_cast<unsigned int>(__popcll(__ballot(1)));                  \
        const int l_ = static_cast<int>(__lane_id());                                              \
        if (__builtin_amdgcn_readfirstlane(l_) == l_) {                                            \
            atomicAdd(&rm_cnt_s[i], 1u);                                                           \
            atomicAdd(&rm_cnt_s[(i) + 16], n_);                                                    \
        }                                                                                          \
    }
__shared__ unsigned int rm_cnt_e[8];
#define RM_CNT_END(i)                                                                              \
    {                                                                                              \
        const unsigned int n_ = static_cast<unsigned int>(__popcll(__ballot(1)));                  \
        const int l_ = static_cast<int>(__lane_id());                                              \
// ... 475 lines not shown
#ifdef RM_STAMPS
    if (dbg_fallback_cycles) *dbg_fallback_cycles += __builtin_amdgcn_s_memtime() - t_fb0;
#endif
    if (fallback) {
        if (!served) closest = all;
        count += static_cast<uint32_t>(S.n_prims);
    } else if (need) {
        count += found;
    }
    return closest;
}

__device__ __forceinline__ int oct_find(const SceneView &S, const Vec3f &p) {
    const RmOctNode *nodes = S.oct;
    if (!box_contains(nodes[0].lo, nodes[0].hi, p)) return -1;
    int i = 0;
    for (;;) {
        const int first = nodes[i].first_child;
        if (first < 0) return i;
        const float cx = nodes[i].center[0], cy = nodes[i].center[1], cz = nodes[i].center[2];
        i = first + (p.x > cx ? 1 : 0) + (p.y > cy ? 2 : 0) + (p.z > cz ? 4 : 0);
    }
}

__device__ double oct_distance_lane(const SceneView &S, int node, const Vec3f &q, uint32_t &count, bool filter) {
    if (node < 0) {
        count += static_cast<uint32_t>(S.n_prims);
        return (filter && S.n_prims >= 2) ? lane_min_filtered(S, nullptr, S.n_prims, q, RM_MAX_DIST)
                                         : lane_min_exact(S, nullptr, S.n_prims, q, RM_MAX_DIST);
    }
    const RmOctNode nd = S.oct[node];
    double closest = RM_MAX_DIST;
    if (nd.prim_count > 0) {
        const int32_t *ids = S.oct_prims + nd.prim_first;
        closest = (filter && nd.prim_count >= 2) ? lane_min_filtered(S, ids, nd.prim_count, q, closest)
                                                : lane_min_exact(S, ids, nd.prim_count, q, closest);
        count += static_cast<uint32_t>(nd.prim_count);
    } else if (nd.is_empty) {
        closest = min_dist(nd.min_distance * 0.99, closest);
    }
    return closest;
}

struct Bundle {
    float n[4][3];
};
__device__ __forceinline__ Bundle make_bundle(const RmRenderParams &C, int x0, int x1, int y0, int y1) {
    const float mu = __builtin_fmaxf(1.0f / static_cast<float>(C.width), 1e-4f);
    const float mv = __builtin_fmaxf(1.0f / static_cast<float>(C.height), 1e-4f);
    const float u0 = (static_cast<float>(x0) / static_cast<float>(C.width) - 0.5f) * 2.0f - mu;
    const float u1 = (static_cast<float>(x1) / static_cast<float>(C.width) - 0.5f) * 2.0f + mu;
    const float v0 = (static_cast<float>(y0) / static_cast<float>(C.height) - 0.5f) * 2.0f - mv;
    const float v1 = (static_cast<float>(y1) / static_cast<float>(C.height) - 0.5f) * 2.0f + mv;
    Bundle b;
#pragma unroll
    for (int k = 0; k < 3; ++k) {
        b.n[0][k] = C.rot[k] + u0 * C.rot[6 + k];
        b.n[1][k] = C.rot[k] + u1 * C.rot[6 + k];
        b.n[2][k] = C.rot[3 + k] + v0 * C.rot[6 + k];
        b.n[3][k] = C.rot[3 + k] + v1 * C.rot[6 + k];
    }
    return b;
}
__device__ __forceinline__ bool bundle_misses_box(const Bundle &b, const float lo[3], const float hi[3], const float o[3]) {
    const float ql[3] = {lo[0] - o[0], lo[1] - o[1], lo[2] - o[2]};
    const float qh[3] = {hi[0] - o[0], hi[1] - o[1], hi[2] - o[2]};
    bool miss = false;
#pragma unroll
    for (int p = 0; p < 4; ++p) {
        float mx = 0.f, mn = 0.f, mag = 0.f;
#pragma unroll
        for (int k = 0; k < 3; ++k) {
            const float a = ql[k] * b.n[p][k], c = qh[k] * b.n[p][k];
            mx += __builtin_fmaxf(a, c);
            mn += __builtin_fminf(a, c);
            mag += __builtin_fmaxf(__builtin_fabsf(a), __builtin_fabsf(c));
        }
        const float tol = 1e-6f * mag;
        miss = miss || ((p & 1) ? mn > tol : mx < -tol);
    }
    return miss;
}

template <bool REL>
__device__ bool bvh_prologue_cull(const SceneView &S, const RmRenderParams &C, const Bundle &B, bool active, const Ray &r,
                                  const RayInv &ri, RayList &L, Interval &first, int lane) {
    bool have = false;
    L.cnt = 0;
    {
        const RmBvhNode root = S.nodes[0];
        double tE = 0.0, tX = 0.0;
        const bool hit = active && node_slab<REL>(S, root, 0, r, ri, tE, tX) && !(tX < 0.0) && !(tE > RM_MAX_DIST);
        if (!__any(hit)) {
            L.live = 0;
            return false;
        }
        active = hit;
    }
    const float o[3] = {C.origin[0], C.origin[1], C.origin[2]};
    for (int j0 = 0; j0 < C.bvh_leaf_count; j0 += 64) {
        const int j = j0 + lane;
        int li = 0;
        bool cand = false;
        if (j < C.bvh_leaf_count) {
            li = C.bvh_leaves[j];
            const RmBvhNode nd = S.nodes[li];
            cand = !bundle_misses_box(B, nd.lo, nd.hi, o);
        }
        unsigned long long m = __ballot(cand);
        while (m) {
            const int src = __builtin_ctzll(m);
            m &= m - 1;
            const int i = __builtin_amdgcn_readlane(li, src);
            RM_CNT(5)
            if (active) {
                const RmBvhNode node = S.nodes[i];
                double tE, tX;
                if (node_slab<REL>(S, node, i, r, ri, tE, tX) && !(tX < 0.0) && !(tE > RM_MAX_DIST)) {
                    const double cE = __builtin_fmax(tE, 0.0);
                    const double cX = __builtin_fmin(tX, RM_MAX_DIST);
                    if (L.cnt < L.cap) L.col[L.cnt * 64] = static_cast<uint16_t>(i);
                    L.cnt++;
                    if (!have || cE < first.tEnter) {
                        first.tEnter = cE;
                        first.tExit = cX;
                        first.ord = i;
                        have = true;
                        L.cur_pos = L.cnt - 1;
                    }
                }
            }
        }
    }
    L.live = L.cnt;
    return have;
}


struct LdsLayout {
    uint32_t nodes, prims, cells, list, oct, oct_prims, spheres, radii, rel, end, step;
};
inline LdsLayout lds_layout_host(const RmRenderParams &C, int accel, bool lds, bool rel) {
    auto up = [](uint32_t v) { return (v + 15u) & ~15u; };
    auto words = [](uint32_t count, uint32_t size) { return ((count * size + 3u) / 4u) * 4u; };
    LdsLayout o = {0, 0, 0, 0, 0, 0, 0, 0, 0, 0, 0};
    uint32_t off = 0;
    if (lds) {
        if (accel == 2) {
            o.nodes = off = up(off);
            off += words(static_cast<uint32_t>(C.bvh_nodes), sizeof(RmBvhNode));
            o.prims = off = up(off);
            off += words(static_cast<uint32_t>(C.bvh_prim_count), 4);
            o.cells = off = up(off);
            off += words(static_cast<uint32_t>(C.pq_cell_count), 4);
            o.list = off = up(off);
            off += words(static_cast<uint32_t>(C.pq_list_count), 2);
        } else if (accel == 1) {
            o.oct = off = up(off);
            off += words(static_cast<uint32_t>(C.oct_nodes), sizeof(RmOctNode));
            o.oct_prims = off = up(off);
            off += words(static_cast<uint32_t>(C.oct_prim_count), 4);
        }
        o.spheres = off = up(off);
        off += words(static_cast<uint32_t>(C.n_prims), sizeof(RmSphere));
        o.radii = off = up(off);
        off += words(static_cast<uint32_t>(C.n_prims), 8);
        off = up(off);
        if (accel == 2 && C.step_box) {
            o.step = off;
            off = up(off + 3u * static_cast<uint32_t>(C.sb_stride) * 4u);
        }
        if (rel) {
            o.rel = off;
            off += static_cast<uint32_t>(C.bvh_nodes) * 48u;
        }
    }
    o.end = off;
    return o;
}
template <int ACCEL, bool LDS, bool REL>
__device__ __forceinline__ LdsLayout lds_layout(const RmRenderParams &C) {
    LdsLayout o;
    o.nodes = C.lds_off[0];
    o.prims = C.lds_off[1];
    o.cells = C.lds_off[2];
    o.list = C.lds_off[3];
    o.oct = C.lds_off[4];
    o.oct_prims = C.lds_off[5];
    o.spheres = C.lds_off[6];
    o.radii = C.lds_off[7];
    o.rel = C.lds_off[8];
    o.end = C.lds_off[9];
// ... 64 lines not shown
};

__device__ __forceinline__ int queue_rows(int tiles_y, int qid) {
    const int x = qid / RM_SUBQ, s = qid % RM_SUBQ;
    const int Rx = (tiles_y - x + 7) >> 3;
    return Rx > s ? (Rx - s + RM_SUBQ - 1) / RM_SUBQ : 0;
}

__device__ __forceinline__ bool queue_entry(const TileQueue &Q, int qid, unsigned int k, int &tile_col, int &tile_row) {
    const int R = queue_rows(Q.tiles_y, qid);
    if (k >= static_cast<unsigned int>(R) * static_cast<unsigned int>(Q.tiles_x)) return false;
    if (Q.perm) k = Q.perm[static_cast<size_t>(qid) * Q.perm_stride + k];
    const unsigned int q = Q.tiles_x_magic ? __umulhi(k, Q.tiles_x_magic) : k;
    const int qi = static_cast<int>(q), mid = R >> 1;
    const int j = (qi & 1) ? mid - ((qi + 1) >> 1) : mid + (qi >> 1);
    tile_row = (qid / RM_SUBQ) + 8 * ((qid % RM_SUBQ) + RM_SUBQ * j);
    tile_col = static_cast<int>(k - q * static_cast<unsigned int>(Q.tiles_x));
    return true;
}
__device__ __forceinline__ unsigned int queue_slot_of(const TileQueue &Q, int qid, int tile_col, int tile_row) {
    const int R = queue_rows(Q.tiles_y, qid), mid = R >> 1;
    const int j = (tile_row >> 3) / RM_SUBQ;
    const int qi = j >= mid ? 2 * (j - mid) : 2 * (mid - j) - 1;
    return static_cast<unsigned int>(qi) * static_cast<unsigned int>(Q.tiles_x) + static_cast<unsigned int>(tile_col);
}

__device__ __forceinline__ bool pull_tile(const TileQueue &Q, int &home, int &tile_col, int &tile_row, int lane,
                                          unsigned int first_claim) {
    unsigned int k = static_cast<unsigned int>(__builtin_amdgcn_readfirstlane(static_cast<int>(first_claim)));
    if (queue_entry(Q, home, k, tile_col, tile_row)) return true;
    const unsigned int mine = static_cast<unsigned int>(queue_rows(Q.tiles_y, lane)) * static_cast<unsigned int>(Q.tiles_x);
    for (int attempt = 0; attempt < 4096; ++attempt) {
        const unsigned int head = __hip_atomic_load(&Q.counters[lane * RM_QSTRIDE], __ATOMIC_RELAXED, __HIP_MEMORY_SCOPE_AGENT);
        const unsigned long long avail = __ballot(head < mine);
        if (avail == 0) return false;
        const int h = (home + 1) & (RM_QUEUES - 1);
        const unsigned long long rot = h ? ((avail >> h) | (avail << (RM_QUEUES - h))) : avail;
        const int x = (h + __builtin_ctzll(rot)) & (RM_QUEUES - 1);
        k = 0;
        if (lane == 0) k = atomicAdd(&Q.counters[x * RM_QSTRIDE], 1u);
        k = static_cast<unsigned int>(__builtin_amdgcn_readfirstlane(static_cast<int>(k)));
        if (queue_entry(Q, x, k, tile_col, tile_row)) {
            home = x;
            return true;
        }
    }
    return false;
}

__device__ __forceinline__ RmRenderParams cold_params() {
#if __HIP_DEVICE_COMPILE__
    typedef const __attribute__((address_space(4))) RmRenderParams *KernArgs;
    KernArgs p = (KernArgs)__builtin_amdgcn_kernarg_segment_ptr();
    asm volatile("" : "+s"(p));
#ifdef RM_RTC_V2
    RmRenderParams r = *p;
    rm_v2_fix(r);
    return r;
#else
    return *p;
#endif
#else
    return RmRenderParams();
#endif
}

template <int ACCEL, bool LDS, bool UR = false, bool REL = false>
__device__ __forceinline__ void render_v2_body(const RmRenderParams &P) {
    extern __shared__ __align__(16) unsigned char smem[];
    __shared__ WaveDiag wave_diag[4];
    const int lane0 = threadIdx.x & 63;
    const int lane = lane0;
    const int wave = __builtin_amdgcn_readfirstlane(static_cast<int>(threadIdx.x >> 6));
    if (lane < 8) {
        wave_diag[wave].sdf[lane] = 0;
        wave_diag[wave].iters[lane] = 0;
        wave_diag[wave].mx[lane] = 0;
        wave_diag[wave].mn_inv[lane] = 0;
    }
#ifdef RM_STAMPS
    if (lane == 0 && P.stamps && blockIdx.x * 4 + wave < 8192) P.stamps[40 + 2 * 8192 + blockIdx.x * 4 + wave] = __builtin_amdgcn_s_memrealtime();
#endif

    {
        const LdsLayout lay = lds_layout<ACCEL, LDS, REL>(P);
        if (LDS) {
            size_t off;
            if (ACCEL == 2) {
                off = lay.nodes;
                stage(smem, off, P.bvh, P.bvh_nodes);
                off = lay.prims;
                stage(smem, off, P.bvh_prims, P.bvh_prim_count);
                off = lay.cells;
                stage(smem, off, P.pq_cells, P.pq_cell_count);
                off = lay.list;
                stage(smem, off, P.pq_list, P.pq_list_count);
            } else if (ACCEL == 1) {
                off = lay.oct;
                stage(smem, off, P.oct, P.oct_nodes);
                off = lay.oct_prims;
                stage(smem, off, P.oct_prims, P.oct_prim_count);
            }
            off = lay.spheres;
            stage(smem, off, P.spheres, P.n_prims);
            off = lay.radii;
            stage(smem, off, P.radii, P.n_prims);
            if (ACCEL == 2) {
                off = lay.step;
                stage(smem, off, P.step_tab, P.step_box ? 3 * P.sb_stride : 0);
            }
            if (REL) {
                double *rel = reinterpret_cast<double *>(smem + lay.rel);
                for (int k = threadIdx.x; k < P.bvh_nodes * 6; k += blockDim.x) {
                    const int node = k / 6, c = k - node * 6;
                    const float v = c < 3 ? P.bvh[node].lo[c] : P.bvh[node].hi[c - 3];
                    rel[k] = static_cast<double>(v) - P.origin_d[c < 3 ? c : c - 3];
                }
            }
            __syncthreads();
        }
    }
    const int list_cap = P.list_cap;
    auto lane_now = []() {
        int l;
        asm volatile("v_mbcnt_lo_u32_b32 %0, -1, 0\n\tv_mbcnt_hi_u32_b32 %0, -1, %0" : "=v"(l));
        return l;
    };
    auto list_column = [&](const RmRenderParams &C) {
        const uint32_t end = C.lds_off[9];
        return reinterpret_cast<uint16_t *>(smem + end) + (static_cast<uint32_t>(wave) * static_cast<uint32_t>(C.list_cap)) * 64u + static_cast<uint32_t>(lane_now());
    };
    const int item_px = P.item_px;
    int home = (P.hw_xcd ? (__builtin_amdgcn_s_getreg(20 | (3 << 11)) & 7) : (static_cast<int>(blockIdx.x) & 7)) * RM_SUBQ +
               static_cast<int>((blockIdx.x >> 3) % RM_SUBQ);
    const int refill_at = P.refill_threshold;

    int tile_col = -1, tile_row = 0, qpos = item_px;
    bool no_more = false;
    unsigned int item_t0 = 0;

    enum : int { ST_PHASE = 7, ST_TRIP_SHIFT = 3, ST_TRIP_MASK = 127 << 3, ST_HAVECUR = 1 << 10, ST_PAR_SHIFT = 11, ST_PAR_MASK = 7 << 11,
                 ST_PIXEL = 1 << 14,
                 ST_LIVE_SHIFT = 15, ST_POS_SHIFT = 22, ST_OVF = 1 << 29, ST_LIST_MASK = (0x3FFF << 15) | (1 << 29) };
    Vec3f rd = {0.f, 0.f, -1.f};
    double inv0 = 0.0, inv1 = 0.0, inv2 = 0.0;
    double t = RM_MAX_DIST;
    double sA = 0.0, sB = 0.0;
    int sC = -1;
    uint32_t counters = 0;
    uint32_t pidx = 0;
    int st = PH_DONE;

    auto ray_of = [&](const RmRenderParams &C) {
        Ray r;
        r.d = rd;
        r.o = {C.origin[0], C.origin[1], C.origin[2]};
        r.od[0] = C.origin_d[0];
        r.od[1] = C.origin_d[1];
        r.od[2] = C.origin_d[2];
        return r;
    };
    auto inv_of = [&]() {
        RayInv ri;
        ri.inv[0] = inv0;
        ri.inv[1] = inv1;
        ri.inv[2] = inv2;
        ri.par[0] = (st & (1 << ST_PAR_SHIFT)) != 0;
        ri.par[1] = (st & (2 << ST_PAR_SHIFT)) != 0;
        ri.par[2] = (st & (4 << ST_PAR_SHIFT)) != 0;
        ri.any_par = (st & ST_PAR_MASK) != 0;
        return ri;
    };
    auto list_of = [&](const RmRenderParams &C) {
        RayList L;
        L.col = list_column(C);
        L.cap = list_cap;
        L.live = (st >> ST_LIVE_SHIFT) & 127;
        L.cur_pos = (st >> ST_POS_SHIFT) & 127;
        L.cnt = (st & ST_OVF) ? list_cap + 1 : L.live;
        return L;
    };
    auto keep_list = [&](const RayList &L) {
        st = (st & ~ST_LIST_MASK) | ((L.live & 127) << ST_LIVE_SHIFT) | ((L.cur_pos & 127) << ST_POS_SHIFT) | (L.cnt > list_cap ? ST_OVF : 0);
    };
    auto set_phase = [&](int ph) { st = (st & ~ST_PHASE) | ph; };
    auto nrm_x = [&]() { return __int_as_float(__double2loint(sB)); };
    auto nrm_y = [&]() { return __int_as_float(__double2hiint(sB)); };
    auto set_normal = [&](float nx, float ny, float nz) {
        sB = __hiloint2double(__float_as_int(ny), __float_as_int(nx));
        sC = __float_as_int(nz);
    };
    auto finish_march = [&](double dist_total) {
        t = dist_total;
        set_phase((t >= RM_MAX_DIST) ? PH_DONE : PH_N0);
    };
    auto store_mine = [&](const RmRenderParams &C) {
        const bool miss = t >= RM_MAX_DIST;
        const float nx = miss ? 0.f : nrm_x(), ny = miss ? 0.f : nrm_y(), nz = miss ? 0.f : __int_as_float(sC);
        store_pixel(C, static_cast<size_t>(pidx), t, nx, ny, nz, counters >> 16, counters & 0xFFFFu);
        if (C.diag_out) wave_diag_add(&wave_diag[wave], lane_now(), counters >> 16, counters & 0xFFFFu);
    };

    RM_T0()
#ifdef RM_STAMPS_LOG
    int refill_k_ = 0;
#endif
#ifdef RM_COUNTS
    if (threadIdx.x < 32) rm_cnt_s[threadIdx.x] = 0;
    if (threadIdx.x < 8) rm_cnt_e[threadIdx.x] = 0;
    __syncthreads();
#endif
    for (;;) {
        RM_T(7)
        RM_CNT(0)
        const unsigned long long idle = __ballot((st & ST_PHASE) == PH_DONE);
        const int n_idle = __popcll(idle);
        if (n_idle >= refill_at || n_idle == 64) {
            RM_CNT(1)
#ifdef RM_STAMPS_LOG
            if (lane == 0 && P.stamps && blockIdx.x * 4 + wave < 2048 && refill_k_ < 96)
                reinterpret_cast<unsigned int *>(P.stamps + 40 + 3 * 8192)[(blockIdx.x * 4 + wave) * 96 + refill_k_] =
                    static_cast<unsigned int>(__builtin_amdgcn_s_memrealtime());
            refill_k_ += 1;
#endif
            const RmRenderParams C = cold_params();
            TileQueue Q;
            Q.counters = C.tile_counters;
            Q.tile_w = C.tile_w;
            Q.item_px = C.item_px;
            Q.tile_h = 1 << C.tile_h_log2;
            Q.tiles_x = C.tiles_x;
            Q.tiles_y = C.tiles_y;
            Q.tiles_x_magic = C.tiles_x_magic;
            Q.perm = C.lpt_perm;
            Q.perm_stride = C.lpt_stride;
            const bool want_tile = !no_more && qpos >= Q.item_px;
            const int lane_r = lane_now();
            if (want_tile) {
                if (C.lpt_cost_out && tile_col >= 0) {
                    const unsigned int took = (static_cast<unsigned int>(__builtin_amdgcn_s_memrealtime()) - item_t0) >> 10;
                    if (lane_r == 0) C.lpt_cost_out[static_cast<size_t>(home) * C.lpt_stride + queue_slot_of(Q, home, tile_col, tile_row)] =
                        static_cast<uint8_t>(took < 255u ? (took ? took : 1u) : 255u);
                }
#ifdef RM_STAMPS_CLAIM
                const unsigned long long tc0 = __builtin_amdgcn_s_memrealtime();
#endif
                unsigned int claim = 0;
                if (lane_r == 0) claim = atomicAdd(&Q.counters[home * RM_QSTRIDE], 1u);
                if (pull_tile(Q, home, tile_col, tile_row, lane_r, claim)) {
                    qpos = 0;
                    if (C.lpt_cost_out) item_t0 = static_cast<unsigned int>(__builtin_amdgcn_s_memrealtime());
                } else no_more = true;
#ifdef RM_STAMPS_CLAIM
                const unsigned long long tc1 = __builtin_amdgcn_s_memrealtime();
                if (lane_r == 0 && P.stamps) {
                    atomicAdd(&P.stamps[38], tc1 - tc0);
                    atomicAdd(&P.stamps[39], 1ull);
                }
#endif
            }
            if ((st & (ST_PHASE | ST_PIXEL)) == (PH_DONE | ST_PIXEL)) {
                store_mine(C);
                st &= ~ST_PIXEL;
            }
            if (!no_more) {
                const int remaining = Q.item_px - qpos;
                const int rank = __builtin_amdgcn_mbcnt_hi(static_cast<unsigned int>(idle >> 32),
                                                           __builtin_amdgcn_mbcnt_lo(static_cast<unsigned int>(idle), 0u));
                const bool take = (st & ST_PHASE) == PH_DONE && rank < remaining;
                bool in_frame = false;
                const bool whole_batch = ACCEL == 2 && C.bvh_leaf_count > 0 && n_idle == 64 && (qpos & 63) == 0;
                const int batch_sub = qpos >> 6;
                Ray ray = ray_of(C);
                RayInv ri = inv_of();
                if (take) {
                    const int n = qpos + rank;
                    const int sub = n >> 6, l = n & 63;
                    const int px = (tile_col << C.item_w_log2) + sub * C.sub_dx + (l & (Q.tile_w - 1));
                    const int prow = (tile_row << C.tile_h_log2) + sub * C.sub_dy + (l >> C.tile_w_log2);
                    if (px < C.width && prow < C.local_rows) {
                        in_frame = true;
                        pidx = static_cast<uint32_t>(prow) * static_cast<uint32_t>(C.width) + static_cast<uint32_t>(px);
                        ray = make_ray(C, px, row_to_y(C, prow));
                        rd = ray.d;
                        counters = 0;
                        t = 0.0;
                        st = PH_MARCH | ST_PIXEL;
                        if (ACCEL == 2) {
                            ri = make_ray_inv(ray);
                            inv0 = ri.inv[0];
                            inv1 = ri.inv[1];
                            inv2 = ri.inv[2];
                            st |= ((ri.par[0] ? 1 : 0) | (ri.par[1] ? 2 : 0) | (ri.par[2] ? 4 : 0)) << ST_PAR_SHIFT;
                        }
                    }
                }
                if (ACCEL == 2) {
#ifdef RM_STAMPS
                    const unsigned long long t_pr0 = __builtin_amdgcn_s_memtime();
#endif
                    RayList L = list_of(C);
                    Interval cur;
                    cur.tEnter = sA;
                    cur.tExit = sB;
                    cur.ord = sC;
                    bool hc = false;
                    if (whole_batch) {
                        const int x0 = (tile_col << C.item_w_log2) + batch_sub * C.sub_dx;
                        const int r0 = (tile_row << C.tile_h_log2) + batch_sub * C.sub_dy;
                        const Bundle B = make_bundle(C, x0, x0 + Q.tile_w - 1, row_to_y(C, r0),
                                                     row_to_y(C, r0 + (64 >> C.tile_w_log2) - 1));
                        hc = bvh_prologue_cull<REL>(scene_view<ACCEL, LDS, REL>(C, smem), C, B, in_frame, ray, ri, L, cur, lane_now());
                    } else if (in_frame) {
                        RM_CNT(15)
                        hc = bvh_prologue<REL>(scene_view<ACCEL, LDS, REL>(C, smem), ray, ri, L, cur);
                    }
#ifdef RM_STAMPS
                    t_acc_[5] += __builtin_amdgcn_s_memtime() - t_pr0;
                    t_prev_ += __builtin_amdgcn_s_memtime() - t_pr0;
#endif
                    if (in_frame) {
                        keep_list(L);
                        if (hc) {
                            sA = cur.tEnter;
                            sB = cur.tExit;
                            sC = cur.ord;
                            st |= ST_HAVECUR;
                        } else {
                            t = RM_MAX_DIST;
                            set_phase(PH_DONE);
                        }
                    }
                }
                qpos += n_idle < remaining ? n_idle : remaining;
            }
        }
        if (no_more && !__any((st & ST_PHASE) != PH_DONE)) {
            if (st & ST_PIXEL) store_mine(cold_params());
            break;
        }
        RM_T(0)

        const RmRenderParams CA = cold_params();
        const SceneView S = scene_view<ACCEL, LDS, REL>(CA, smem);
        const Ray ray = ray_of(CA);
        bool need = false;
        Vec3f q = {0.f, 0.f, 0.f};
        int onode = -1;
        if ((st & ST_PHASE) == PH_MARCH) {
            for (;;) {
                if ((st & ST_TRIP_MASK) >= (RM_MAX_STEPS << ST_TRIP_SHIFT)) {
                    finish_march(t);
                    break;
                }
                st += 1 << ST_TRIP_SHIFT;
                RM_CNT(2)
                const Vec3f p = point_at(ray, t);
                if (ACCEL == 2) {
                    double skip = 0.0;
                    bool terminate = !(st & ST_HAVECUR);
                    if (!terminate) {
                        if (t < sA) skip = sA - t;
                        else if (t > sB) {
                            RayList L = list_of(CA);
                            Interval cur;
                            cur.tEnter = sA;
                            cur.tExit = sB;
                            cur.ord = sC;
                            const bool hc = bvh_next<REL>(S, ray, inv_of(), L, sA, sC, cur);
                            keep_list(L);
                            if (!hc) {
                                st &= ~ST_HAVECUR;
                                terminate = true;
                            } else {
                                sA = cur.tEnter;
                                sB = cur.tExit;
                                sC = cur.ord;
                                if (sA > t) skip = sA - t;
                            }
                        }
                    }
                    if (terminate) {
                        finish_march(RM_MAX_DIST);
                        break;
                    }
                    if (skip > 0.0) {
                        t += skip;
                        if (t > RM_MAX_DIST) {
                            finish_march(t);
                            break;
                        }
                        continue;
                    }
                } else if (ACCEL == 1) {
                    onode = oct_find(S, p);
// ... 356 lines not shown
        cost[e] = c;
        sum += c;
        nz += c != 0;
    }
    atomicAdd(&sum_s, sum);
    atomicAdd(&nz_s, nz);
    __syncthreads();
    const float mean = nz_s ? static_cast<float>(sum_s) / static_cast<float>(nz_s) : 1e9f;
    auto cls = [&](uint8_t c) { const float f = c; return f >= 4.f * mean ? 0 : (f >= 2.f * mean ? 1 : (f >= 1.25f * mean ? 2 : 3)); };
    const int chunk = (n + 1023) / 1024, e0 = threadIdx.x * chunk, e1 = min(n, e0 + chunk);
    unsigned int mine[4] = {0, 0, 0, 0};
    for (int e = e0; e < e1; ++e) mine[cls(cost[e])]++;
    for (int c = 0; c < 4; ++c) cnt[c * 1024 + threadIdx.x] = mine[c];
    __syncthreads();
    if (threadIdx.x < 4) {
        unsigned int run = 0;
        for (int t = 0; t < 1024; ++t) {
            const unsigned int v = cnt[threadIdx.x * 1024 + t];
            cnt[threadIdx.x * 1024 + t] = run;
            run += v;
        }
        base_s[threadIdx.x] = run;
    }
    __syncthreads();
    unsigned int start[4], acc = 0;
    for (int c = 0; c < 4; ++c) {
        start[c] = acc + cnt[c * 1024 + threadIdx.x];
        acc += base_s[c];
    }
    for (int e = e0; e < e1; ++e) {
        const int c = cls(cost[e]);
        perm[static_cast<size_t>(x) * stride + start[c]++] = static_cast<uint16_t>(e);
    }
}
}
hipError_t rm_launch_lpt_sort(const uint8_t *cost_prev, uint16_t *perm, int stride, int tiles_x, int tiles_y, hipStream_t stream) {
    const size_t shmem = static_cast<size_t>((stride + 15) & ~15) + 4 * 1024 * sizeof(unsigned int);
    hipLaunchKernelGGL(lpt_sort_kernel, dim3(RM_QUEUES), dim3(1024), shmem, stream, cost_prev, perm, stride, tiles_x, tiles_y);
    return hipGetLastError();
}
#endif

hipError_t RM_LEN_VARIANT(rm_launch_wave_distance)(const RmRenderParams &p, const float *points, int64_t n, double *dist, uint32_t *count, hipStream_t stream) {
    if (p.accel != 2 || p.general || p.bvh_nodes <= 0) return hipErrorInvalidValue;
    if (n <= 0) return hipSuccess;
    const dim3 grid(static_cast<unsigned>((n + 255) / 256)), block(256);
    if (p.uniform_radius) hipLaunchKernelGGL(wave_distance_kernel<true>, grid, block, 0, stream, p, points, n, dist, count);
    else hipLaunchKernelGGL(wave_distance_kernel<false>, grid, block, 0, stream, p, points, n, dist, count);
    return hipGetLastError();
}

hipError_t RM_LEN_VARIANT(rm_launch_render_v2)(const RmRenderParams &p_in, hipStream_t stream, const char **kernel_name, uint32_t *shape) {
    RmRenderParams p = p_in;
    const int rows = p.local_rows;
    if (kernel_name) *kernel_name = "";
    if (rows <= 0 || p.width <= 0) return hipSuccess;
    if (!p.tile_counters) return hipErrorInvalidValue;
    if (p.leaf_order) p.bvh_prim_count = 0;
    if (p.item_px != 64 && p.item_px != 128 && p.item_px != 256) p.item_px = 64;
    if (p.item_px < p.tile_w) p.item_px = p.tile_w;
    const int tw = p.tile_w;
    const bool wide = p.item_wide != 0 && tw < 64 && p.item_px > 64;
    const int iw = wide ? tw * (p.item_px / 64) : tw, th = wide ? 64 / tw : p.item_px / tw;
    const int tiles_x = (p.width + iw - 1) / iw;
    const int tiles_y = (rows + th - 1) / th;
    auto log2i = [](int v) { int l = 0; while ((1 << l) < v) ++l; return l; };
    if ((tw & (tw - 1)) != 0 || tiles_x <= 0 || static_cast<long long>(tiles_x) * (tiles_y + 8) >= (1ll << 31)) return hipErrorInvalidValue;
    p.tile_w_log2 = log2i(tw);
    p.tile_h_log2 = log2i(th);
    p.item_w_log2 = log2i(iw);
    p.sub_dx = wide ? tw : 0;
    p.sub_dy = wide ? 0 : 64 / tw;
    p.tiles_x = tiles_x;
    p.tiles_y = tiles_y;
    p.tiles_x_magic = tiles_x == 1 ? 0u : static_cast<uint32_t>((1ull << 32) / static_cast<unsigned long long>(tiles_x)) + 1u;
    const unsigned needed = static_cast<unsigned>((static_cast<long long>(tiles_x) * tiles_y + 3) / 4);
    unsigned resident = 0, blocks = 0;
    if (p.refill_threshold < 1) p.refill_threshold = 1;
    if (p.refill_threshold > 64) p.refill_threshold = 64;
    const RmV2Plan plan = rm_v2_plan(p);
    const bool lds = plan.lds, rel = plan.rel;
    p.list_cap = plan.list_cap;
    p.step_box = plan.step_box;
    const size_t list_bytes = plan.list_bytes, scene_bytes = plan.scene_bytes, rel_bytes = static_cast<size_t>(p.bvh_nodes) * 48;
    size_t shmem = (lds ? scene_bytes : 0) + (rel ? rel_bytes + 16 : 0) + list_bytes + 16;
    if (p.lds_fill && p.blocks_per_cu >= 2 && p.blocks_per_cu <= 8) {
        const size_t room = (160 * 1024 / static_cast<size_t>(p.blocks_per_cu)) / 1280 * 1280 - sizeof(WaveDiag) * 4;
        if (room > shmem && room <= 64 * 1024) shmem = room;
    }
    {
        const LdsLayout lay = lds_layout_host(p, p.accel, lds, rel && p.accel == 2);
        const uint32_t v[11] = {lay.nodes, lay.prims, lay.cells, lay.list, lay.oct, lay.oct_prims, lay.spheres, lay.radii, lay.rel, lay.end, lay.step};
        for (int k = 0; k < 11; ++k) p.lds_off[k] = v[k];
        if (lay.end + list_bytes > shmem) return hipErrorInvalidValue;
    }
    const int cus = p.num_cus > 0 ? p.num_cus : 256;
    const int floor_per_cu = p.launch_per_cu > 0 ? p.launch_per_cu : p.blocks_per_cu;
    const int per_cu = rm_v2_overlap_per_cu(floor_per_cu, p.overlap_per_cu, static_cast<long long>(tiles_x) * tiles_y, cus);
    resident = static_cast<unsigned>(cus) * static_cast<unsigned>(per_cu > 0 ? per_cu : 4);
    blocks = needed < resident ? (needed ? needed : 1u) : resident;
    if (shape) {
        shape[0] = blocks;
        shape[1] = 256;
        shape[2] = static_cast<uint32_t>(shmem);
        shape[3] = p.step_box ? 1u : 0u;
    }
    hipError_t e = hipSuccess;
    if (!p.diag_block) e = hipMemsetAsync(p.tile_counters, 0, RM_QUEUES * RM_QSTRIDE * sizeof(unsigned int), stream);
    if (e != hipSuccess) return e;
    p.lpt_perm = nullptr;
    if (p.lpt_perm_out) {
        const long long per_queue = static_cast<long long>(queue_rows_host(tiles_y, 0)) * tiles_x;
        if (per_queue <= p.lpt_stride && per_queue <= 32768) {
            e = rm_launch_lpt_sort(p.lpt_cost_prev, p.lpt_perm_out, p.lpt_stride, tiles_x, tiles_y, stream);
            if (e != hipSuccess) return e;
            p.lpt_perm = p.lpt_perm_out;
        } else {
            p.lpt_cost_out = nullptr;
        }
    } else {
        p.lpt_cost_out = nullptr;
    }
    const dim3 grid(blocks), block(256);
#define RM_V2X(A, L, U, R)                                                                                                   \
    {                                                                                                                        \
        const void *fn_ = p.rtc_ctx ? rm_rtc_v2_hook(p, A, L, U, R, RM_LEN_IS_SQRT) : nullptr;                               \
        if (fn_) {                                                                                                           \
            size_t bytes_ = sizeof p;                                                                                        \
            void *extra_[] = {HIP_LAUNCH_PARAM_BUFFER_POINTER, &p, HIP_LAUNCH_PARAM_BUFFER_SIZE, &bytes_, HIP_LAUNCH_PARAM_END}; \
            e = hipModuleLaunchKernel(reinterpret_cast<hipFunction_t>(const_cast<void *>(fn_)), grid.x, 1, 1, 256, 1, 1,     \
                                      static_cast<unsigned>(shmem), stream, nullptr, extra_);                               \
            if (e != hipSuccess) return e;                                                                                   \
            if (kernel_name) *kernel_name = "render_kernel_v2<" #A ", " #L ", " #U ", " #R ">" RM_LEN_TAG " [launch constants compiled in]"; \
        } else {                                                                                                             \
            hipLaunchKernelGGL((render_kernel_v2<A, L, U, R>), grid, block, shmem, stream, p);                               \
            if (kernel_name) *kernel_name = "render_kernel_v2<" #A ", " #L ", " #U ", " #R ">" RM_LEN_TAG;                   \
        }                                                                                                                    \
    }
#define RM_V2(A, L) RM_V2X(A, L, false, false)
    if (p.accel == 2) {
        if (lds && rel && p.uniform_radius) RM_V2X(2, true, true, true)
        else if (lds && rel) RM_V2X(2, true, false, true)
        else if (lds && p.uniform_radius) RM_V2X(2, true, true, false)
        else if (lds) RM_V2(2, true)
        else RM_V2(2, false)
    }
    else if (p.accel == 1) { if (lds) RM_V2(1, true) else RM_V2(1, false) }
    else { if (lds) RM_V2(0, true) else RM_V2(0, false) }
#undef RM_V2X
#undef RM_V2
    return hipGetLastError();
}
#endif
```

### cpu_raymarcher_amd/csrc/rm_rtc.cpp

```cpp
#include "rm_rtc.h"

#include "rm_v2_fields.h"

#include <dlfcn.h>
#include <hip/hip_runtime_api.h>
#include <hip/hiprtc.h>

#include <algorithm>
#include <chrono>
#include <cmath>
#include <cstdio>
#include <cstdlib>
#include <cstring>
#include <map>
#include <mutex>
#include <thread>

#define RM_EMBED(sym, file)                                                                                   \
    __asm__(".pushsection .rodata\n .hidden " #sym "\n .global " #sym "\n" #sym ":\n .incbin \"" file "\"\n .byte 0\n .popsection\n"); \
    extern "C" const char sym[];
RM_EMBED(rm_src_kernels_hip, "rm_kernels.hip")
RM_EMBED(rm_src_render_v2_hip, "rm_render_v2.hip")
RM_EMBED(rm_src_device_h, "rm_device.h")
RM_EMBED(rm_src_jsmath_h, "rm_jsmath.h")
// ... 358 lines not shown
        const int first = bvh[i].leaf >> 8, cnt = bvh[i].leaf & 0xFF;
        if (cnt == 0) continue;
        if (first < 0 || static_cast<size_t>(first) + static_cast<size_t>(cnt) > prims.size()) return false;
        for (int j = 0; j < cnt; ++j)
            if (prims[first + j] < 0 || prims[first + j] >= n_obj) return false;
        leaves.push_back(i);
        listed += cnt;
    }
    if (leaves.empty() || leaves.size() > 8 || listed > 32) return false;
    for (int i = 0; i < n; ++i) {
        for (int k = 0; k < 3; ++k)
            if (!std::isfinite(bvh[i].lo[k]) || !std::isfinite(bvh[i].hi[k])) return false;
        if (parent[i] >= 0)
            for (int k = 0; k < 3; ++k)
                if (!(bvh[i].lo[k] >= bvh[parent[i]].lo[k] && bvh[i].hi[k] <= bvh[parent[i]].hi[k])) return false;
    }
    auto box = [&](int i) {
        const RmBvhNode &nd = bvh[i];
        return "const float lo[3] = {" + lit_f(nd.lo[0]) + ", " + lit_f(nd.lo[1]) + ", " + lit_f(nd.lo[2]) + "}, hi[3] = {" + lit_f(nd.hi[0]) + ", " + lit_f(nd.hi[1]) +
               ", " + lit_f(nd.hi[2]) + "};";
    };
    out += "#define RM_RTC_BVH_LEAVES " + std::to_string(leaves.size()) + "\n";
    out += "__device__ __forceinline__ bool rm_rtc_bvh_next_interval(const Ray &r, const RayInv &ri, double keyT, int keyOrd, Interval &out) {\n    bool have = false;\n";
    for (int i : leaves) {
        out += "    {  // node " + std::to_string(i) + "\n        " + box(i) + "\n        double tE, tX;\n";
        out += "        if (slab_inv(lo, hi, r, ri, tE, tX) && !(tX < 0.0) && !(tE > RM_MAX_DIST)) {  // bvh.ts:145,151\n";
        out += "            const double cE = tE > 0.0 ? tE : 0.0, cX = tX < RM_MAX_DIST ? tX : RM_MAX_DIST;\n";
        out += "            const bool after = cE > keyT || (cE == keyT && " + std::to_string(i) + " > keyOrd);\n";
        out += "            const bool better = !have || cE < out.tEnter;\n";
        out += "            if (after && better) {\n                out.tEnter = cE;\n                out.tExit = cX;\n                out.ord = " + std::to_string(i) +
               ";\n                have = true;\n            }\n        }\n    }\n";
    }
    out += "    return have;\n}\n";
    out += "__device__ __forceinline__ double rm_rtc_bvh_distance(const Vec3f &p, double time, uint32_t &count) {\n    double closest = RM_MAX_DIST;\n    uint32_t found = 0;\n";
    for (int i : leaves) {
        const int first = bvh[i].leaf >> 8, cnt = bvh[i].leaf & 0xFF;
        out += "    {  // node " + std::to_string(i) + "\n        " + box(i) + "\n        if (box_contains(lo, hi, p)) {\n";
        for (int j = 0; j < cnt; ++j)
            out += "            closest = js_min_nan(rm_rtc_obj_" + std::to_string(prims[first + j]) + "(p.x, p.y, p.z, time), closest);\n";
        out += "            found += " + std::to_string(cnt) + "u;\n        }\n    }\n";
    }
    out += "    if (found == 0) {\n";
    for (int r = 0; r < n_obj; ++r) out += "        closest = js_min_nan(rm_rtc_obj_" + std::to_string(r) + "(p.x, p.y, p.z, time), closest);\n";
    out += "        found = " + std::to_string(n_obj) + "u;\n    }\n    count += found;\n    return closest;\n}\n";
    return true;
}

}

std::string scene_source(const std::vector<RmInstr> &prog, const std::vector<int32_t> &obj_ranges, const std::vector<rmh::ProgTreeNode> &tree,
                         const std::vector<int32_t> &roots, bool prune, const std::vector<RmBvhNode> &bvh, const std::vector<int32_t> &bvh_prims, bool require_bvh) {
    const int n_obj = static_cast<int>(obj_ranges.size() / 2);
    if (n_obj < 1 || n_obj > kMaxObjects || prog.size() > static_cast<size_t>(kMaxInstructions) || roots.size() != static_cast<size_t>(n_obj)) return std::string();
    std::string out = "// generated by rm_rtc.cpp: the scene's expression trees, one function per object\nnamespace rmd {\n";
    for (int r = 0; r < n_obj; ++r)
        if (roots[r] < 0 || roots[r] >= static_cast<int>(tree.size()) || !emit_object(prog, tree, roots[r], r, prune, out)) return std::string();
    out += "__device__ __forceinline__ double rm_rtc_object_sdf(int obj, const Vec3f &p, double time) {\n    switch (obj) {\n";
    for (int r = 0; r < n_obj; ++r)
        out += "        case " + std::to_string(r) + ": return rm_rtc_obj_" + std::to_string(r) + "(p.x, p.y, p.z, time);\n";
    out += "        default: return 0.0;\n    }\n}\n";
    std::string tree_code;
    if (emit_bvh(bvh, bvh_prims, n_obj, tree_code)) out += tree_code;
    else if (require_bvh && !bvh.empty()) return std::string();
    out += "}  // namespace rmd\n";
    return out;
}

bool available(std::string *why) {
    Rtc &r = rtc();
    if (!r.lib && why) *why = r.why;
    return r.lib != nullptr;
}

namespace {

struct Unit {
    std::string defines;
    const char *main_file;
    const char *gen_name;
    const std::string *gen;
    const char *render_fn;
    const char *distance_fn;
    std::string display;
    bool no_scratch;
};

long remark_of(const std::string &log, const char *fn, const char *key) {
    size_t at = log.find(std::string("Function Name: ") + fn);
    if (at == std::string::npos) return -1;
    const size_t next = log.find("Function Name: ", at + 15);
    at = log.find(std::string(key) + ": ", at);
    if (at == std::string::npos || (next != std::string::npos && at > next)) return -1;
    return std::strtol(log.c_str() + at + std::strlen(key) + 2, nullptr, 10);
}

bool compile_unit(const Unit &u, bool load_module, Kernel &out, std::string &log) {
    Rtc &r = rtc();
    if (!r.lib) {
        log = r.why;
        return false;
    }
    std::string extra;
    if (const char *env = std::getenv("RM_RTC_DEFINES")) {
        std::string word;
        for (const char *c = env;; ++c) {
            if (*c && *c != ' ') word += *c;
            else {
                if (!word.empty()) extra += "#define " + word + " 1\n";
                word.clear();
                if (!*c) break;
            }
        }
    }
    const std::string main_src = extra + u.defines + "#include \"" + u.main_file + "\"\n";
    const char *names[] = {"rm_kernels.hip", "rm_render_v2.hip", "rm_device.h", "rm_jsmath.h", "rm_types.h", "rm_program.h", "rm_bvh_list.h", "rm_kernels.h",
                           "rm_diag.h", u.gen_name};
    const char *texts[] = {rm_src_kernels_hip, rm_src_render_v2_hip, rm_src_device_h, rm_src_jsmath_h, rm_src_types_h, rm_src_program_h, rm_src_bvh_list_h,
                           rm_src_kernels_h, rm_src_diag_h, u.gen->c_str()};
    hiprtcProgram prog = nullptr;
    if (r.create(&prog, main_src.c_str(), "rm_rtc_main.hip", 10, texts, names) != HIPRTC_SUCCESS) {
        log = "hiprtcCreateProgram failed";
        return false;
    }
    std::vector<const char *> opts = {"--offload-arch=gfx950", "-O3", "-std=c++17", "-ffp-contract=off", "-fno-fast-math", "-mllvm", "-amdgpu-inline-max-bb=100000"};
    opts.push_back("-Rpass-analysis=kernel-resource-usage");
    const auto t0 = std::chrono::steady_clock::now();
    const hiprtcResult res = r.compile(prog, static_cast<int>(opts.size()), opts.data());
    out.compile_seconds = std::chrono::duration<double>(std::chrono::steady_clock::now() - t0).count();
    size_t ls = 0;
    r.log_size(prog, &ls);
    log.assign(ls, '\0');
    if (ls) r.log(prog, &log[0]);
    while (!log.empty() && log.back() == '\0') log.pop_back();
    if (res != HIPRTC_SUCCESS) {
        r.destroy(&prog);
        if (log.empty()) log = "hiprtcCompileProgram failed";
        return false;
    }
    for (const char *fn : {u.render_fn, u.distance_fn}) {
        if (!fn) continue;
        const long spills = remark_of(log, fn, "VGPRs Spill"), scratch = remark_of(log, fn, "ScratchSize [bytes/lane]");
        if (spills != 0 || (u.no_scratch && scratch != 0)) {
            r.destroy(&prog);
            log = "refused: " + std::string(fn) + " spills " + std::to_string(spills) + " VGPRs, " + std::to_string(scratch) + " bytes of scratch per lane\n" + log;
            return false;
        }
    }
    size_t cs = 0;
    r.code_size(prog, &cs);
    std::vector<char> code(cs);
    r.code(prog, code.data());
    r.destroy(&prog);
    out.name = u.display;
    out.log = log;
    if (!load_module) return true;
    hipModule_t mod = nullptr;
    hipFunction_t fr = nullptr, fd = nullptr;
    if (hipModuleLoadData(&mod, code.data()) != hipSuccess) {
        log += "\nhipModuleLoadData failed";
        (void)hipGetLastError();
        return false;
    }
    if (hipModuleGetFunction(&fr, mod, u.render_fn) != hipSuccess || (u.distance_fn && hipModuleGetFunction(&fd, mod, u.distance_fn) != hipSuccess)) {
        log += "\nthe compiled module lacks its kernels";
        (void)hipGetLastError();
        (void)hipModuleUnload(mod);
        return false;
    }
    out.module = mod;
    out.render = fr;
    out.distance = fd;
    return true;
}

template <typename T>
std::string lit_of(T v) { return std::to_string(v); }
template <>
std::string lit_of<uint32_t>(uint32_t v) { return std::to_string(v) + "u"; }
template <>
std::string lit_of<float>(float v) { return lit_f(v); }
template <>
std::string lit_of<double>(double v) { return lit_d(v); }

}

bool compile(const std::string &scene_src, int accel, bool other, bool length_sqrt, bool load_module, Kernel &out, std::string &log) {
    if (scene_src.empty()) {
        log = "no specialised source for this scene";
        return false;
    }
    Unit u;
    u.defines = "#define RM_RTC 1\n#define RM_RTC_ACCEL " + std::to_string(accel == 1 || accel == 2 ? accel : 0) + "\n#define RM_RTC_OTHER " + (other ? "1" : "0") + "\n" +
                (length_sqrt ? "#define RM_LENGTH_SQRT 1\n" : "");
    u.main_file = "rm_kernels.hip";
    u.gen_name = "rm_rtc_scene.inc";
    u.gen = &scene_src;
    u.render_fn = "rm_rtc_render";
    u.distance_fn = "rm_rtc_distance";
    u.display = std::string("rm_rtc_render<") + std::to_string(accel) + ", " + (other ? "true" : "false") + ">" + (length_sqrt ? " [length=sqrt]" : "");
    u.no_scratch = false;
    return compile_unit(u, load_module, out, log);
}

std::string v2_fixed_source(const RmRenderParams &p, bool with_counts) {
    std::string s = "// generated by rm_rtc.cpp: the configuration parameters of one launch of the v2 wave loop (rm_v2_fields.h)\n"
                    "__device__ __forceinline__ void rm_v2_fix(RmRenderParams &C) {\n";
#define RM_X(f) s += "    C." #f " = " + lit_of(p.f) + ";\n";
    RM_V2_FIXED_SCALARS(RM_X)
    if (with_counts) {
        RM_V2_FIXED_COUNTS(RM_X)
    }
#undef RM_X
#define RM_X(f, n) \
    for (int k = 0; k < n; ++k) s += "    C." #f "[" + std::to_string(k) + "] = " + lit_of(p.f[k]) + ";\n";
    RM_V2_FIXED_ARRAYS(RM_X)
#undef RM_X
    return s + "}\n";
}

uint64_t v2_fixed_hash(const RmRenderParams &p, int variant_bits) {
    uint64_t h = 1469598103934665603ull ^ static_cast<uint64_t>(variant_bits);
    auto mix = [&](const void *d, size_t n) {
        const unsigned char *b = static_cast<const unsigned char *>(d);
        for (size_t i = 0; i < n; ++i) h = (h ^ b[i]) * 1099511628211ull;
    };
#define RM_X(f) mix(&p.f, sizeof p.f);
    RM_V2_FIXED_SCALARS(RM_X)
    RM_V2_FIXED_COUNTS(RM_X)
#undef RM_X
#define RM_X(f, n) mix(p.f, sizeof p.f);
    RM_V2_FIXED_ARRAYS(RM_X)
#undef RM_X
    return h;
}

bool compile_v2(const std::string &fixed_src, int accel, bool lds, bool ur, bool rel, bool length_sqrt, bool load_module, Kernel &out, std::string &log) {
    Unit u;
    u.defines = "#define RM_RTC_V2 1\n#define RM_RTC_V2_ACCEL " + std::to_string(accel) + "\n#define RM_RTC_V2_LDS " + (lds ? "1" : "0") + "\n#define RM_RTC_V2_UR " +
                (ur ? "1" : "0") + "\n#define RM_RTC_V2_REL " + (rel ? "1" : "0") + "\n" + (length_sqrt ? "#define RM_LENGTH_SQRT 1\n" : "");
    u.main_file = "rm_render_v2.hip";
    u.gen_name = "rm_v2_fixed.inc";
    u.gen = &fixed_src;
    u.render_fn = "rm_rtc_render_v2";
    u.distance_fn = nullptr;
    u.display = "rm_rtc_render_v2";
    u.no_scratch = true;
    return compile_unit(u, load_module, out, log);
}

namespace {
struct Cache {
    std::mutex mu;
    std::map<std::string, Kernel> done;
    std::map<std::string, std::string> failed;
    std::map<std::string, bool> running;
};
Cache &cache() {
    static Cache *c = new Cache();
    return *c;
}
std::string cache_key(int device, const std::string &scene_src, int accel, bool other, bool length_sqrt) {
    const char *env = std::getenv("RM_RTC_DEFINES");
    return std::to_string(device) + "|" + std::to_string(accel) + (other ? "|o" : "|s") + (length_sqrt ? "|q|" : "|h|") + (env ? env : "") + "|" + scene_src;
}
bool compile_any(const std::string &src, int accel, bool other, bool length_sqrt, Kernel &out, std::string &log) {
    if (accel & kV2Bit) return compile_v2(src, accel & 3, (accel >> 2) & 1, (accel >> 3) & 1, (accel >> 4) & 1, length_sqrt, true, out, log);
    return compile(src, accel, other, length_sqrt, true, out, log);
}
int lookup(Cache &c, const std::string &key, Kernel &out, std::string &log) {
    auto it = c.done.find(key);
    if (it != c.done.end()) {
        out = it->second;
        out.compile_seconds = 0;
        log = out.log;
        return 1;
    }
    auto f = c.failed.find(key);
    if (f != c.failed.end()) {
        log = f->second;
        return -1;
    }
    return 0;
}
}

bool compile_cached(int device, const std::string &scene_src, int accel, bool other, bool length_sqrt, Kernel &out, std::string &log, bool *cached) {
    Cache &c = cache();
    const std::string key = cache_key(device, scene_src, accel, other, length_sqrt);
    std::lock_guard<std::mutex> lock(c.mu);
    if (const int known = lookup(c, key, out, log)) {
        if (cached) *cached = known > 0;
        return known > 0;
    }
    if (!compile_any(scene_src, accel, other, length_sqrt, out, log)) {
        if (out.name.empty() && c.failed.size() < static_cast<size_t>(kCacheEntries)) c.failed[key] = log;
        return false;
    }
    const bool keep = c.done.size() < static_cast<size_t>(kCacheEntries);
    if (keep) c.done.emplace(key, out);
    if (cached) *cached = keep;
    return true;
}

int compile_async(int device, const std::string &scene_src, int accel, bool other, bool length_sqrt, Kernel &out, std::string &log) {
    Cache &c = cache();
    const std::string key = cache_key(device, scene_src, accel, other, length_sqrt);
    {
        std::lock_guard<std::mutex> lock(c.mu);
        if (const int known = lookup(c, key, out, log)) return known;
        if (c.running.count(key)) return 0;
        if (c.done.size() >= static_cast<size_t>(kCacheEntries)) {
            log = "the kernel cache is full";
            return -1;
        }
        c.running[key] = true;
    }
    std::thread([key, device, scene_src, accel, other, length_sqrt] {
        Kernel k;
        std::string text;
        const bool ok = hipSetDevice(device) == hipSuccess && compile_any(scene_src, accel, other, length_sqrt, k, text);
        Cache &cc = cache();
        std::lock_guard<std::mutex> lock(cc.mu);
        if (ok && !cc.done.count(key)) cc.done.emplace(key, k);
        else if (!ok) cc.failed[key] = text;
        cc.running.erase(key);
    }).detach();
    return 0;
}

void release(Kernel &k) {
    if (k.module) (void)hipModuleUnload(static_cast<hipModule_t>(k.module));
    k = Kernel();
}

}
```

### cpu_raymarcher_amd/csrc/rm_rtc.h

```cpp
#pragma once
#include <string>
#include <vector>

#include "rm_scene_host.h"
#include "rm_types.h"

namespace rmrtc {

struct Kernel {
    void *module = nullptr;
    void *render = nullptr;
    void *distance = nullptr;
    std::string name;
    double compile_seconds = 0;
    std::string log;
};

constexpr int kMaxObjects = 32, kMaxInstructions = 512;
std::string scene_source(const std::vector<RmInstr> &prog, const std::vector<int32_t> &obj_ranges, const std::vector<rmh::ProgTreeNode> &tree,
                         const std::vector<int32_t> &roots, bool prune, const std::vector<RmBvhNode> &bvh, const std::vector<int32_t> &bvh_prims,
                         bool require_bvh);

bool available(std::string *why);

bool compile(const std::string &scene_src, int accel, bool other, bool length_sqrt, bool load_module, Kernel &out, std::string &log);
void release(Kernel &k);

std::string v2_fixed_source(const RmRenderParams &p, bool with_counts);
uint64_t v2_fixed_hash(const RmRenderParams &p, int variant_bits);
bool compile_v2(const std::string &fixed_src, int accel, bool lds, bool ur, bool rel, bool length_sqrt, bool load_module, Kernel &out, std::string &log);
constexpr int kV2Bit = 1 << 8;

constexpr int kCacheEntries = 256;
bool compile_cached(int device, const std::string &scene_src, int accel, bool other, bool length_sqrt, Kernel &out, std::string &log, bool *cached);
int compile_async(int device, const std::string &scene_src, int accel, bool other, bool length_sqrt, Kernel &out, std::string &log);

}
```

### cpu_raymarcher_amd/csrc/rm_types.h

```cpp
#pragma once
#ifndef __HIPCC_RTC__
#include <stdint.h>
#else
using __hip_internal::int8_t;
using __hip_internal::int16_t;
using __hip_internal::int32_t;
using __hip_internal::int64_t;
using __hip_internal::uint8_t;
using __hip_internal::uint16_t;
using __hip_internal::uint32_t;
using __hip_internal::uint64_t;
#endif

struct RmBvhNode {
    float lo[3];
    int32_t skip;
    float hi[3];
    int32_t leaf;
};

struct RmOctNode {
    float lo[3];
    int32_t first_child;
    float hi[3];
    int32_t prim_first;
    double min_distance;
    int32_t prim_count;
    int32_t is_empty;
    float center[3];
    int32_t sub_first;
};

#define RM_OCT_SUB 12

struct RmOctFrameNode {
    double lo[3];
    double cap;
    double hi[3];
    double pad;
};

struct RmSphere {
    float cx, cy, cz;
    float rf;
};

struct RmSphereRec {
    float cx, cy, cz, rf;
    double radius;
    int32_t id, pad;
};

struct RmPrim {
    float m[16];
    int32_t type;
    float half[3];
    double a, b;
};

struct RmInstr {
    float T[16];
    float Tinv[16];
    double p[6];
    int32_t op, src, dst;
    int32_t flags;
};
#define RM_PROG_MAX_SLOTS 16
#define RM_PROG_MAX_VALS 16

#define RM_BVH_LEAF_MAX 255
#define RM_MAX_STEPS 100
#define RM_MAX_DIST 10.0
#define RM_EPSILON 0.001

struct RmDiagBlock;
struct RmFrameDiagBlock;
struct RmDiagDevice;

struct RmFrameView {
    float rot[9];
    float origin[3];
    double origin_d[3];
    double time;
};

#define RM_V2_WAVES 6

struct RmRenderParams {
    int32_t width, height, y_start, y_end;
    float rot[9];
    float origin[3];
    float light[3];
    double rot_d[9], origin_d[3], light_d[3];
    int32_t n_prims;
    int32_t accel;
    int32_t shader;
    int32_t bvh_nodes;
    int32_t oct_nodes;
    int32_t tile_w;
    int32_t nodes_in_lds;
    int32_t filter;
    int32_t variant;
    int32_t list_cap;
    int32_t coop;
    int32_t bvh_prim_count;
    int32_t oct_prim_count;
    int32_t blocks_per_cu;
    int32_t num_cus;
    int32_t pq_dim[3];
    int32_t pq_cell_count;
    int32_t pq_list_count;
    int32_t use_grid;
    float pq_origin[3];
    float pq_inv[3];
    float pq_cell[3];
    int32_t refill_threshold;
    int32_t hw_xcd;
    int32_t item_px;
    int32_t local_rows;
    int32_t stripe_rows;
    int32_t n_parts, part;
    int32_t rel_boxes;
    const uint16_t *lpt_perm;
    uint8_t *lpt_cost_out;
    const uint8_t *lpt_cost_prev;
    uint16_t *lpt_perm_out;
    int32_t lpt_stride;
    int32_t launch_per_cu;
    int32_t v1_lists;
    int32_t v1_list_offset;
    uint32_t lds_off[11];
    int32_t prim_filter;
    int32_t n0_batch;
    const int32_t *stripe_ids;
    unsigned int *tile_counters;
    unsigned long long *stamps;
    const uint32_t *pq_cells;
    const uint16_t *pq_list;
    const uint16_t *bvh_leaves;
    int32_t bvh_leaf_count;
    int32_t v1_block;
    int32_t oct_lean;
    const uint32_t *nn_cells;
    const uint16_t *nn_list;
    int32_t nn_cell_count, nn_list_count, use_nn;
    int32_t tile_w_log2, tile_h_log2, tiles_x, tiles_y;
    int32_t item_wide, item_w_log2, sub_dx, sub_dy;
    const void *rtc_function;
    void *rtc_ctx;
    uint32_t tiles_x_magic;
    int32_t lds_budget_kb;
    int32_t leaf_order;
    int32_t nn_dim[3];
    float nn_inv[3];
    int32_t overlap_per_cu;
    const uint32_t *ext_cells;
    const uint16_t *ext_list;
    int32_t ext_dim[3];
    float ext_origin[3], ext_inv[3];
    int32_t use_ext;
    int32_t algorithm;
    int32_t general;
    int32_t uniform_radius;
    const RmPrim *prims;
    const RmInstr *prog;
    const int32_t *obj_ranges;
    int32_t prog_slots, prog_vals;
    double time;
    double overshoot;
    double step_size;
    const RmSphere *spheres;
    const double *radii;
    const RmBvhNode *bvh;
    const int32_t *bvh_prims;
    const RmOctNode *oct;
    const int32_t *oct_prims;
    const RmSphereRec *oct_recs;
    const int32_t *oct_lut;
    const RmOctFrameNode *oct_frame;
    const uint32_t *oct_sub_hdr;
    const uint8_t *oct_sub_list;
    uint8_t *depth;
    uint8_t *normal;
    uint16_t *sdf;
    uint16_t *iters;
    uint8_t *rgba;
    int32_t lds_fill;
    int32_t multi_step;
    RmDiagBlock *diag_block;
    RmDiagDevice *diag_out;
    const uint32_t *step_tab;
    float sb_origin[3], sb_inv[3];
    int32_t sb_bins, sb_stride;
    int32_t step_box;
};
```

### cpu_raymarcher_amd/csrc/rm_v2_fields.h

```cpp
#pragma once

#define RM_V2_FIXED_SCALARS(X)                                                                                                  \
    X(width) X(height) X(accel) X(shader) X(tile_w) X(nodes_in_lds) X(filter) X(variant) X(list_cap) X(coop) X(use_grid)         \
    X(refill_threshold) X(hw_xcd) X(item_px) X(rel_boxes) X(lpt_stride) X(prim_filter) X(n0_batch) X(use_nn) X(tile_w_log2)     \
    X(tile_h_log2) X(tiles_x) X(item_wide) X(item_w_log2) X(sub_dx) X(sub_dy) X(tiles_x_magic) X(leaf_order) X(algorithm)       \
    X(general) X(uniform_radius) X(multi_step) X(use_ext) X(step_box) X(sb_bins) X(sb_stride)

#define RM_V2_FIXED_COUNTS(X)                                                                                                    \
    X(n_prims) X(bvh_nodes) X(oct_nodes) X(bvh_prim_count) X(oct_prim_count) X(pq_cell_count) X(pq_list_count) X(bvh_leaf_count) \
    X(nn_cell_count) X(nn_list_count)

#define RM_V2_FIXED_ARRAYS(X) \
    X(pq_dim, 3) X(lds_off, 11) X(nn_dim, 3) X(pq_origin, 3) X(pq_inv, 3) X(pq_cell, 3) X(nn_inv, 3) X(light, 3) X(light_d, 3) \
    X(ext_dim, 3) X(ext_origin, 3) X(ext_inv, 3) X(sb_origin, 3) X(sb_inv, 3)
```

### include/rm_raymarch.h

```cpp
#ifndef RM_RAYMARCH_H
#define RM_RAYMARCH_H

#include <stddef.h>
#include <stdint.h>

#ifdef __cplusplus
extern "C" {
#endif

#define RM_API __attribute__((visibility("default")))

typedef struct rm_ctx rm_ctx;

typedef enum rm_status {
    RM_OK = 0,
    RM_E_INVALID = -1,
    RM_E_UNSUPPORTED = -2,
    RM_E_NO_DEVICE = -3,
    RM_E_HIP = -4,
    RM_E_NO_SCENE = -5,
    RM_E_NOMEM = -6
} rm_status;

typedef enum rm_accel { RM_ACCEL_NONE = 0, RM_ACCEL_OCTREE = 1, RM_ACCEL_BVH = 2 } rm_accel;
// ... 294 lines not shown
                                  void *d_rgba, void *stream);
RM_API int rm_shade_ranged(rm_ctx *ctx, int32_t counter, int32_t width, int32_t rows, int32_t n_frames,
                           const uint16_t *values, const rm_frame_hist *hist, uint32_t lo, uint32_t hi,
                           uint8_t *rgba);

RM_API int rm_shade_lit_device(rm_ctx *ctx, int32_t width, int32_t rows, int32_t n_frames, const void *d_depth,
                               const void *d_normal, const void *d_lit, const void *d_ao, void *d_rgba, void *stream);
RM_API int rm_shade_lit(rm_ctx *ctx, int32_t width, int32_t rows, int32_t n_frames, const uint8_t *depth,
                        const uint8_t *normal, const float *lit, const float *ao, uint8_t *rgba);

typedef enum rm_field_map { RM_FIELD_MAP_DISTANCE = 0, RM_FIELD_MAP_COUNT = 1 } rm_field_map;
typedef struct rm_field_shade {
    int32_t  map, reserved;
    double   range;
    double   band;
    double   line;
    uint32_t lo, hi;
} rm_field_shade;
RM_API int rm_shade_field_device(rm_ctx *ctx, const rm_field_shade *shade, int64_t n, const void *d_values, void *d_rgba,
                                 void *stream);
RM_API int rm_shade_field(rm_ctx *ctx, const rm_field_shade *shade, int64_t n, const void *values, uint8_t *rgba);

RM_API int rm_render_stripes_device(rm_ctx *ctx, const rm_job *job, int32_t shader, int32_t stripe_rows,
                                    int32_t n_parts, int32_t part, void *d_depth, void *d_normal,
                                    void *d_sdf, void *d_iters, void *d_rgba, void *stream);
RM_API int rm_stripe_rows(int32_t y_start, int32_t y_end, int32_t stripe_rows, int32_t n_parts, int32_t part);

RM_API int rm_deal_stripes(int32_t rows, int32_t stripe_rows, int32_t n_parts, const int32_t *weights, int32_t *owner);

RM_API int rm_render_stripe_list_device(rm_ctx *ctx, const rm_job *job, int32_t shader, int32_t stripe_rows,
                                        const int32_t *stripe_ids, int32_t n_stripes, void *d_depth, void *d_normal,
                                        void *d_sdf, void *d_iters, void *d_rgba, void *stream);

RM_API int rm_assemble_frame_device(rm_ctx *ctx, const void *d_gathered, int64_t rank_stride, int64_t section_offset,
                                    int32_t row_bytes, int32_t height, int32_t stripe_rows, const int32_t *owner,
                                    int32_t n_stripes, int32_t world, void *d_frame, int64_t acc_offset, void *d_acc,
                                    void *stream);

RM_API int rm_shade(rm_ctx *ctx, int32_t shader, int32_t width, int32_t height,
                    const uint8_t *depth, const uint8_t *normal, const uint16_t *sdf,
                    const uint16_t *iters, uint8_t *rgba);
RM_API int rm_shade_device(rm_ctx *ctx, int32_t shader, int32_t width, int32_t height,
                           const void *d_depth, const void *d_normal, const void *d_sdf,
                           const void *d_iters, void *d_rgba, void *stream);

RM_API int rm_reduce_counters(rm_ctx *ctx, const uint16_t *sdf, const uint16_t *iters, int64_t n,
                              rm_diagnostics *out);
RM_API int rm_reduce_counters_device(rm_ctx *ctx, const void *d_sdf, const void *d_iters, int64_t n,
                                     rm_diagnostics *out, void *stream);

RM_API int rm_reduce_counters_enqueue(rm_ctx *ctx, const void *d_sdf, const void *d_iters, int64_t n,
                                      void *d_acc, void *stream);

RM_API int rm_render_attach_diagnostics(rm_ctx *ctx, void *d_acc);


RM_API int rm_partition_rows(int32_t height, int32_t n_workers, int32_t i, int32_t *y_start,
                             int32_t *y_end);


RM_API int rm_selftest_hypot(rm_ctx *ctx, const float *xyz, int64_t n, double *out);

RM_API int rm_selftest_jsmath(rm_ctx *ctx, int32_t fn, const double *a, const double *b, int64_t n, double *out);

RM_API int rm_selftest_hypot64(rm_ctx *ctx, const double *xyz, int64_t n, int32_t on_device, double *out);

RM_API int rm_selftest_fastdiv(rm_ctx *ctx, uint64_t seed, int64_t n, uint64_t *mismatches);

RM_API int rm_selftest_recip(rm_ctx *ctx, int mode, uint64_t *mismatches);

RM_API int rm_debug_read_stamps(rm_ctx *ctx, uint64_t *out8);

RM_API int rm_rtc_source(rm_ctx *ctx, char *out, int64_t cap, int64_t *needed);
RM_API int rm_rtc_compile_check(rm_ctx *ctx, int32_t accel, int32_t other, char *log, int64_t cap, double *seconds);
RM_API int rm_rtc_status(rm_ctx *ctx, int32_t *compiled, int32_t *failed, char *log, int64_t cap);

RM_API int rm_debug_read_counts(rm_ctx *ctx, uint64_t *out32);
RM_API int rm_debug_read_lpt_costs(rm_ctx *ctx, uint8_t *out, int64_t n);
RM_API int rm_debug_scene_table(rm_ctx *ctx, const char *name, int32_t from_device, void *out, int64_t cap, int64_t *bytes);
RM_API int rm_debug_launch_fill(rm_ctx *ctx, int32_t asked, int32_t *effective);
RM_API int rm_debug_last_launch(rm_ctx *ctx, uint32_t out[4]);
RM_API int rm_debug_overlap_fill(rm_ctx *ctx, int32_t asked, int64_t items, int32_t *effective);
RM_API int rm_debug_step_box(rm_ctx *ctx, int32_t out[6]);
RM_API int rm_debug_read_wave_times(rm_ctx *ctx, uint64_t *out24576);
RM_API int rm_debug_read_batch_log(rm_ctx *ctx, uint32_t *out196608);

RM_API int rm_set_option(rm_ctx *ctx, const char *key, int64_t value);
RM_API int rm_get_option(const rm_ctx *ctx, const char *key, int64_t *value);

#ifdef __cplusplus
}
#endif
#endif
```

Before: 1666.

## Cull BVH leaves per tile using projected screen-space leaf rectangles

Each block projects the BVH leaf boxes to pixel-space rectangles once per launch, storing them in a per-launch device buffer. The per-tile prologue cull then uses a cheap integer rectangle-overlap test instead of the ray-bundle/box test, and skips the root slab test. Tiles with no candidate leaves can skip the prologue entirely. It also adds a fallback recompile with machine LICM disabled when kernel compilation fails. In exchange, every block recomputes the rectangles, and the projection is conservative, so it may keep more candidates than the bundle test.

Measured after the change: 1706 (median of 6 runs). 1.02x the previous value.

```diff
diff --git a/cpu_raymarcher_amd/_native.py b/cpu_raymarcher_amd/_native.py
--- a/cpu_raymarcher_amd/_native.py
+++ b/cpu_raymarcher_amd/_native.py
@@ -243,6 +243,8 @@
     "rm_debug_last_launch": (C.c_int, [_VP, C.POINTER(C.c_uint32)]),
     "rm_debug_overlap_fill": (C.c_int, [_VP, C.c_int32, C.c_int64, C.POINTER(C.c_int32)]),
     "rm_debug_step_box": (C.c_int, [_VP, C.POINTER(C.c_int32)]),
+    "rm_debug_rect_cull": (C.c_int, [_VP, _VP, _VP, C.c_int32, C.c_int32, C.POINTER(C.c_int32)]),
+    "rm_debug_leaf_rects": (C.c_int, [_VP, _VP, _VP, C.c_int32, C.c_int32, _VP, _VP, C.c_int64, C.POINTER(C.c_int64)]),
     "rm_rtc_source": (C.c_int, [_VP, C.c_char_p, C.c_int64, C.POINTER(C.c_int64)]),
     "rm_rtc_compile_check": (C.c_int, [_VP, C.c_int32, C.c_int32, C.c_char_p, C.c_int64, C.POINTER(C.c_double)]),
     "rm_rtc_status": (C.c_int, [_VP, C.POINTER(C.c_int32), C.POINTER(C.c_int32), C.c_char_p, C.c_int64]),
diff --git a/cpu_raymarcher_amd/context.py b/cpu_raymarcher_amd/context.py
--- a/cpu_raymarcher_amd/context.py
+++ b/cpu_raymarcher_amd/context.py
@@ -156,6 +156,24 @@
         out = (C.c_int32 * 6)()
         N.check(self._h, N.lib().rm_debug_step_box(self._h, out))
         return dict(last=bool(out[0]), planned=bool(out[1]), reason=out[2], list_cap=out[3], list_cap_without=out[4], table_bytes=out[5])
+
+    def rect_cull(self, rot, origin, width, height):
+        r = np.ascontiguousarray(rot, dtype=np.float32).reshape(9)
+        o = np.ascontiguousarray(origin, dtype=np.float32).reshape(3)
+        out = (C.c_int32 * 5)()
+        N.check(self._h, N.lib().rm_debug_rect_cull(self._h, _ptr(r), _ptr(o), int(width), int(height), out))
+        return dict(last=bool(out[0]), planned=bool(out[1]), reason=out[2], leaves=out[3], max_leaves=out[4])
+
+    def leaf_rects(self, rot, origin, width, height):
+        r = np.ascontiguousarray(rot, dtype=np.float32).reshape(9)
+        o = np.ascontiguousarray(origin, dtype=np.float32).reshape(3)
+        n = C.c_int64(0)
+        N.check(self._h, N.lib().rm_debug_leaf_rects(self._h, _ptr(r), _ptr(o), int(width), int(height), None, None, 0, C.byref(n)))
+        rects = np.zeros((max(1, n.value), 4), np.uint16)
+        nodes = np.zeros(max(1, n.value), np.int32)
+        N.check(self._h, N.lib().rm_debug_leaf_rects(self._h, _ptr(r), _ptr(o), int(width), int(height), _ptr(rects), _ptr(nodes),
+                                                     n.value, C.byref(n)))
+        return rects[:n.value], nodes[:n.value]
 
     def scene_from_preset(self, index, accel):
         N.check(self._h, N.lib().rm_scene_from_preset(self._h, int(index), int(accel)))
diff --git a/cpu_raymarcher_amd/csrc/rm_api.cpp b/cpu_raymarcher_amd/csrc/rm_api.cpp
--- a/cpu_raymarcher_amd/csrc/rm_api.cpp
+++ b/cpu_raymarcher_amd/csrc/rm_api.cpp
@@ -50,6 +50,7 @@
     static constexpr unsigned kLaunches = 1024, kHeads = 64, kHeadWords = 64;
     unsigned int *heads = nullptr;
     RmDiagBlock *blocks = nullptr;
+    RmLeafRect *rects = nullptr;
     unsigned int head_slot = 0, block_slot = 0;
 
     hipError_t init() {
@@ -57,12 +58,15 @@
         hipError_t e = hipMalloc(reinterpret_cast<void **>(&heads), head_bytes);
         if (e == hipSuccess) e = hipMemset(heads, 0, head_bytes);
         if (e == hipSuccess) e = hipMalloc(reinterpret_cast<void **>(&blocks), block_bytes);
-        return e == hipSuccess ? hipMemset(blocks, 0, block_bytes) : e;
+        if (e == hipSuccess) e = hipMemset(blocks, 0, block_bytes);
+        return e == hipSuccess ? hipMalloc(reinterpret_cast<void **>(&rects), sizeof(RmLeafRect) * kLaunches * RM_RECT_CULL_MAX_LEAVES) : e;
     }
     void release() {
         (void)hipFree(heads);
         (void)hipFree(blocks);
-    }
+        (void)hipFree(rects);
+    }
+    RmLeafRect *rects_of_last_heads() { return rects && head_slot ? rects + static_cast<size_t>(RM_RECT_CULL_MAX_LEAVES) * ((head_slot - 1) % kLaunches) : nullptr; }
     unsigned int *take_heads() { return heads ? heads + static_cast<size_t>(kHeads) * kHeadWords * (head_slot++ % kLaunches) : nullptr; }
     RmDiagBlock *take_block() { return blocks ? blocks + block_slot++ % kLaunches : nullptr; }
 };
@@ -362,7 +366,7 @@
     int64_t opt_min_fill = 1;
     int64_t opt_overlap_fill = 1;
     int hw_queues = 4;
-    uint32_t last_v2_shape[4] = {0, 0, 0, 0};
+    uint32_t last_v2_shape[5] = {0, 0, 0, 0, 0};
     int64_t opt_item_wide = 0;
     int64_t opt_multi_step = 1;
     int64_t opt_step_box = 1;
@@ -372,6 +376,8 @@
     int64_t opt_static = 0;
     int64_t opt_lut = 1;
     int64_t opt_cull = 1;
+    int64_t opt_rect_cull = 1;
+    std::vector<uint16_t> cull_leaves;
     int64_t opt_rel = 1;
     int64_t opt_uniform = 1;
     int64_t opt_sub = 1;
@@ -486,7 +492,8 @@
     if (e.state < 0) return nullptr;
     if (e.state == 0 && ++e.launches < ctx->opt_v2_after) return nullptr;
     for (;;) {
-        const int st = obtain_kernel(ctx, rmrtc::v2_fixed_source(p, !e.lite), bits, false, length_sqrt, e.k);
+        int st = obtain_kernel(ctx, rmrtc::v2_fixed_source(p, !e.lite), bits, false, length_sqrt, e.k);
+        if (st < 0) st = obtain_kernel(ctx, rmrtc::v2_fixed_source(p, !e.lite), bits | rmrtc::kV2NoLicmBit, false, length_sqrt, e.k);
         e.state = st > 0 ? 1 : (st < 0 ? -1 : 2);
         if (st >= 0 || e.lite) break;
         e.lite = true;
@@ -511,6 +518,8 @@
     p.oct_frame = oct_table ? oct_table->dev : nullptr;
     if (ctx->opt_lpt && v2) ctx->lpt.acquire(p);
     if (v2 && !empty) p.tile_counters = ctx->slots.take_heads();
+    p.leaf_rects = v2 && !empty && p.rect_cull ? ctx->slots.rects_of_last_heads() : nullptr;
+    if (!p.leaf_rects) p.rect_cull = 0;
     p.diag_out = diag_out;
     RmDiagDevice *reduce_after = nullptr;
     if (p.diag_out && !v2 && !empty && p.sdf && p.iters) {
@@ -627,6 +636,7 @@
         if (rmh::leaf_objects(ctx->host, prog, ranges, tree, roots))
             ctx->rtc_src = rmrtc::scene_source(prog, ranges, tree, roots, false, ctx->host.bvh, ctx->host.bvh_prims, true);
     }
+    ctx->cull_leaves = cull_leaf_table(ctx->host.bvh);
     if (!ctx->has_device) {
         free_device_scene(ctx);
         return RM_OK;
@@ -640,9 +650,8 @@
     if ((always || !ctx->host.name.empty()) && (rc = upload_vec(ctx, ctx->host.name, &ctx->dev.name))) return rc;
     RM_SCENE_ARRAYS(RM_X)
 #undef RM_X
-    const std::vector<uint16_t> leaves = cull_leaf_table(ctx->host.bvh);
-    ctx->dev.bvh_leaf_count = static_cast<int32_t>(leaves.size());
-    return upload_vec(ctx, leaves, &ctx->dev.bvh_leaves);
+    ctx->dev.bvh_leaf_count = static_cast<int32_t>(ctx->cull_leaves.size());
+    return upload_vec(ctx, ctx->cull_leaves, &ctx->dev.bvh_leaves);
 }
 
 int clamp_preset(int idx) { return idx < 0 ? 0 : (idx > rmh::kPresetCount - 1 ? rmh::kPresetCount - 1 : idx); }
@@ -986,6 +995,14 @@
         return hipEventRecord(ctx->scratch_busy, user);
     }
 };
+
+int rect_cull_refusal(const rm_ctx *ctx, const float rot[9], const float origin[3], int32_t width, int32_t height) {
+    if (!ctx->opt_rect_cull || !ctx->opt_cull || ctx->host.accel != RM_ACCEL_BVH) return 1;
+    if (ctx->cull_leaves.size() > RM_RECT_CULL_MAX_LEAVES || (ctx->cull_leaves.empty() && ctx->host.bvh_leaves > RM_RECT_CULL_MAX_LEAVES)) return 2;
+    if (ctx->cull_leaves.empty()) return 1;
+    if (!rm_rect_cull_camera_ok(rot, origin) || width < 1 || height < 1 || width > 65536 || height > 65536) return 3;
+    return 0;
+}
 
 int fill_params(rm_ctx *ctx, const rm_job *job, RmRenderParams &p) {
     if (!job) return fail(ctx, RM_E_INVALID, "null job");
@@ -1057,6 +1074,7 @@
     p.pq_list = ctx->dev.pq_list;
     p.bvh_leaves = ctx->dev.bvh_leaves;
     p.bvh_leaf_count = (ctx->opt_cull && ctx->host.accel == RM_ACCEL_BVH) ? ctx->dev.bvh_leaf_count : 0;
+    p.rect_cull = rect_cull_refusal(ctx, p.rot, p.origin, p.width, p.height) == 0 ? 1 : 0;
     p.nn_cells = ctx->dev.nn_cells;
     p.nn_list = ctx->dev.nn_list;
     p.nn_cell_count = static_cast<int32_t>(ctx->host.nn_cells.size());
@@ -2903,6 +2921,54 @@
     const bool v2 = p.variant == 2 && p.algorithm == 0 && p.accel == 2;
     out[1] = v2 && plan.step_box ? 1 : 0;
     out[2] = out[1] ? 0 : (ctx->host.step_tab.empty() && v2 && ctx->opt_step_box && ctx->opt_multi_step ? 2 : (v2 && plan.refused ? 3 : 1));
+    return RM_OK;
+}
+
+int rm_debug_rect_cull(rm_ctx *ctx, const float *rot9, const float *origin3, int32_t width, int32_t height, int32_t out[5]) {
+    if (!ctx || !out || !rot9 || !origin3) return RM_E_INVALID;
+    for (int k = 0; k < 5; ++k) out[k] = 0;
+    out[0] = static_cast<int32_t>(ctx->last_v2_shape[4]);
+    out[4] = RM_RECT_CULL_MAX_LEAVES;
+    if (!ctx->have_scene) return fail(ctx, RM_E_NO_SCENE, "no scene set");
+    rm_job job;
+    std::memset(&job, 0, sizeof job);
+    job.width = job.height = job.y_end = 64;
+    job.algorithm = RM_ALG_SPHERE_TRACER;
+    job.scene_preset_index = ctx->scene_is_uploaded ? RM_SCENE_UPLOADED : ctx->scene_preset;
+    job.acceleration_structure = ctx->host.accel;
+    job.overshoot_factor = job.step_size = std::nan("");
+    const double scene_time = ctx->time;
+    RmRenderParams p;
+    const int rc = fill_params(ctx, &job, p);
+    ctx->time = scene_time;
+    if (rc) return rc;
+    out[3] = static_cast<int32_t>(ctx->cull_leaves.size());
+    const bool v2 = p.variant == 2 && p.algorithm == 0 && p.accel == 2;
+    out[2] = v2 ? rect_cull_refusal(ctx, rot9, origin3, width, height) : 1;
+    out[1] = out[2] == 0 ? 1 : 0;
+    return RM_OK;
+}
+
+int rm_debug_leaf_rects(rm_ctx *ctx, const float *rot9, const float *origin3, int32_t width, int32_t height, uint16_t *rects,
+                        int32_t *nodes, int64_t cap, int64_t *n) {
+    if (!ctx || !n || !rot9 || !origin3 || cap < 0) return RM_E_INVALID;
+    *n = 0;
+    int32_t why[5];
+    const int rc = rm_debug_rect_cull(ctx, rot9, origin3, width, height, why);
+    if (rc) return rc;
+    if (!why[1]) return RM_OK;
+    *n = static_cast<int64_t>(ctx->cull_leaves.size());
+    for (int64_t j = 0; j < *n && j < cap; ++j) {
+        const RmBvhNode &nd = ctx->host.bvh[ctx->cull_leaves[static_cast<size_t>(j)]];
+        const RmLeafRect r = rm_leaf_rect(nd.lo, nd.hi, origin3, rot9, width, height);
+        if (rects) {
+            rects[4 * j] = r.x_lo;
+            rects[4 * j + 1] = r.x_hi;
+            rects[4 * j + 2] = r.y_lo;
+            rects[4 * j + 3] = r.y_hi;
+        }
+        if (nodes) nodes[j] = ctx->cull_leaves[static_cast<size_t>(j)];
+    }
     return RM_OK;
 }
 
@@ -2941,6 +3007,7 @@
     {"min_fill", &rm_ctx::opt_min_fill, kSwitch, {}, nullptr},
     {"overlap_fill", &rm_ctx::opt_overlap_fill, kSwitch, {}, nullptr},
     {"cull", &rm_ctx::opt_cull, kSwitch, {}, nullptr},
+    {"rect_cull", &rm_ctx::opt_rect_cull, kSwitch, {}, nullptr},
     {"rel", &rm_ctx::opt_rel, kSwitch, {}, nullptr},
     {"static", &rm_ctx::opt_static, kRange, {0, 95}, "static must be in [0, 95] percent"},
     {"sub", &rm_ctx::opt_sub, kSwitch, {}, nullptr},
diff --git a/cpu_raymarcher_amd/csrc/rm_kernels.h b/cpu_raymarcher_amd/csrc/rm_kernels.h
--- a/cpu_raymarcher_amd/csrc/rm_kernels.h
+++ b/cpu_raymarcher_amd/csrc/rm_kernels.h
@@ -23,6 +23,44 @@
 #define RM_LEN_TAG ""
 #define RM_LEN_IS_SQRT false
 #endif
+
+inline __host__ __device__ RmLeafRect rm_leaf_rect(const float lo[3], const float hi[3], const float o[3], const float rot[9], int W, int H) {
+    const RmLeafRect whole = {0, 65535, 0, 65535}, none = {65535, 0, 65535, 0};
+    double ql[3], qh[3];
+    for (int k = 0; k < 3; ++k) {
+        ql[k] = static_cast<double>(lo[k]) - static_cast<double>(o[k]);
+        qh[k] = static_cast<double>(hi[k]) - static_cast<double>(o[k]);
+    }
+    double umin = 0.0, umax = 0.0, vmin = 0.0, vmax = 0.0;
+    bool behind = false;
+#pragma unroll 1
+    for (int corner = 0; corner < 8; ++corner) {
+        const double qx = (corner & 1) ? qh[0] : ql[0], qy = (corner & 2) ? qh[1] : ql[1], qz = (corner & 4) ? qh[2] : ql[2];
+        const double z = -(qx * rot[6] + qy * rot[7] + qz * rot[8]);
+        const double a = qx * rot[0] + qy * rot[1] + qz * rot[2];
+        const double b = qx * rot[3] + qy * rot[4] + qz * rot[5];
+        if (!(z > 1e-6 * (__builtin_fabs(qx) + __builtin_fabs(qy) + __builtin_fabs(qz)))) behind = true;
+        const double u = a / z, v = b / z;
+        if (corner == 0 || u < umin) umin = u;
+        if (corner == 0 || u > umax) umax = u;
+        if (corner == 0 || v < vmin) vmin = v;
+        if (corner == 0 || v > vmax) vmax = v;
+    }
+    if (behind) return whole;
+    const double mu = __builtin_fmax(1.0 / W, 1e-4), mv = __builtin_fmax(1.0 / H, 1e-4);
+    const double xl = ((umin - mu - 1e-6 * (1.0 + __builtin_fabs(umin))) * 0.5 + 0.5) * W;
+    const double xh = ((umax + mu + 1e-6 * (1.0 + __builtin_fabs(umax))) * 0.5 + 0.5) * W;
+    const double yl = ((vmin - mv - 1e-6 * (1.0 + __builtin_fabs(vmin))) * 0.5 + 0.5) * H;
+    const double yh = ((vmax + mv + 1e-6 * (1.0 + __builtin_fabs(vmax))) * 0.5 + 0.5) * H;
+    if (!(xl - xl == 0.0 && xh - xh == 0.0 && yl - yl == 0.0 && yh - yh == 0.0)) return whole;
+    if (xh < 0.0 || yh < 0.0 || xl > W - 1.0 || yl > H - 1.0) return none;
+    RmLeafRect r;
+    r.x_lo = static_cast<uint16_t>(xl <= 0.0 ? 0 : (xl >= 65535.0 ? 65535 : static_cast<int>(__builtin_floor(xl))));
+    r.x_hi = static_cast<uint16_t>(xh >= 65535.0 ? 65535 : static_cast<int>(__builtin_ceil(xh)));
+    r.y_lo = static_cast<uint16_t>(yl <= 0.0 ? 0 : (yl >= 65535.0 ? 65535 : static_cast<int>(__builtin_floor(yl))));
+    r.y_hi = static_cast<uint16_t>(yh >= 65535.0 ? 65535 : static_cast<int>(__builtin_ceil(yh)));
+    return r;
+}
 
 enum { RM_CMP_NONE = -1, RM_CMP_SDF = 0, RM_CMP_ITERS = 1, RM_CMP_DEPTH = 2, RM_CMP_NORMAL = 3, RM_CMP_SURFACE = 4 };
 struct RmCompareStats {
@@ -205,6 +243,19 @@
     return items >= RM_V2_OVERLAP_ITEMS_PER_WAVE * waves ? candidate : floor_per_cu;
 }
 
+inline bool rm_rect_cull_camera_ok(const float rot[9], const float origin[3]) {
+    for (int k = 0; k < 3; ++k)
+        if (!(origin[k] - origin[k] == 0.f)) return false;
+    for (int i = 0; i < 3; ++i)
+        for (int j = i; j < 3; ++j) {
+            double d = 0.0;
+            for (int k = 0; k < 3; ++k) d += static_cast<double>(rot[3 * i + k]) * static_cast<double>(rot[3 * j + k]);
+            const double err = d - (i == j ? 1.0 : 0.0);
+            if (!(err >= -1e-6 && err <= 1e-6)) return false;
+        }
+    return true;
+}
+
 struct RmV2Plan {
     bool lds, rel;
     int list_cap, step_box, tier, refused;
diff --git a/cpu_raymarcher_amd/csrc/rm_render_v2.hip b/cpu_raymarcher_amd/csrc/rm_render_v2.hip
--- a/cpu_raymarcher_amd/csrc/rm_render_v2.hip
+++ b/cpu_raymarcher_amd/csrc/rm_render_v2.hip
@@ -581,12 +581,17 @@
     return miss;
 }
 
+__device__ __forceinline__ bool rect_overlaps(const RmLeafRect &q, int x0, int x1, int y0, int y1) {
+    return x0 <= static_cast<int>(q.x_hi) && x1 >= static_cast<int>(q.x_lo) && y0 <= static_cast<int>(q.y_hi) && y1 >= static_cast<int>(q.y_lo);
+}
+
 template <bool REL>
-__device__ bool bvh_prologue_cull(const SceneView &S, const RmRenderParams &C, const Bundle &B, bool active, const Ray &r,
+__device__ bool bvh_prologue_cull(const SceneView &S, const RmRenderParams &C, int x0, int x1, int y0, int y1, bool rect,
+                                  unsigned long long cand0, bool active, const Ray &r,
                                   const RayInv &ri, RayList &L, Interval &first, int lane) {
     bool have = false;
     L.cnt = 0;
-    {
+    if (!rect) {
         const RmBvhNode root = S.nodes[0];
         double tE = 0.0, tX = 0.0;
         const bool hit = active && node_slab<REL>(S, root, 0, r, ri, tE, tX) && !(tX < 0.0) && !(tE > RM_MAX_DIST);
@@ -597,16 +602,22 @@
         active = hit;
     }
     const float o[3] = {C.origin[0], C.origin[1], C.origin[2]};
+    Bundle B = {};
+    if (!rect) B = make_bundle(C, x0, x1, y0, y1);
     for (int j0 = 0; j0 < C.bvh_leaf_count; j0 += 64) {
         const int j = j0 + lane;
         int li = 0;
         bool cand = false;
         if (j < C.bvh_leaf_count) {
             li = C.bvh_leaves[j];
-            const RmBvhNode nd = S.nodes[li];
-            cand = !bundle_misses_box(B, nd.lo, nd.hi, o);
-        }
-        unsigned long long m = __ballot(cand);
+            if (!rect) {
+                const RmBvhNode nd = S.nodes[li];
+                cand = !bundle_misses_box(B, nd.lo, nd.hi, o);
+            } else if (j0 != 0) {
+                cand = rect_overlaps(C.leaf_rects[j], x0, x1, y0, y1);
+            }
+        }
+        unsigned long long m = rect && j0 == 0 ? cand0 : __ballot(cand);
         while (m) {
             const int src = __builtin_ctzll(m);
             m &= m - 1;
@@ -837,6 +848,15 @@
     if (lane == 0 && P.stamps && blockIdx.x * 4 + wave < 8192) P.stamps[40 + 2 * 8192 + blockIdx.x * 4 + wave] = __builtin_amdgcn_s_memrealtime();
 #endif
 
+    if (ACCEL == 2 && P.rect_cull) {
+        const float o[3] = {P.origin[0], P.origin[1], P.origin[2]};
+        const float rot[9] = {P.rot[0], P.rot[1], P.rot[2], P.rot[3], P.rot[4], P.rot[5], P.rot[6], P.rot[7], P.rot[8]};
+        for (int j = threadIdx.x; j < P.bvh_leaf_count && j < RM_RECT_CULL_MAX_LEAVES; j += blockDim.x) {
+            const RmBvhNode nd = P.bvh[P.bvh_leaves[j]];
+            P.leaf_rects[j] = rm_leaf_rect(nd.lo, nd.hi, o, rot, P.width, P.height);
+        }
+        if (!LDS) __syncthreads();
+    }
     {
         const LdsLayout lay = lds_layout<ACCEL, LDS, REL>(P);
         if (LDS) {
@@ -991,6 +1011,9 @@
             Q.perm_stride = C.lpt_stride;
             const bool want_tile = !no_more && qpos >= Q.item_px;
             const int lane_r = lane_now();
+            const bool rect_batch = ACCEL == 2 && C.rect_cull && n_idle == 64;
+            RmLeafRect rect0 = {65535, 0, 65535, 0};
+            if (rect_batch && lane_r < C.bvh_leaf_count) rect0 = C.leaf_rects[lane_r];
             if (want_tile) {
                 if (C.lpt_cost_out && tile_col >= 0) {
                     const unsigned int took = (static_cast<unsigned int>(__builtin_amdgcn_s_memrealtime()) - item_t0) >> 10;
@@ -1014,6 +1037,18 @@
                 }
 #endif
             }
+            const bool rect_cull_now = rect_batch && !no_more && (qpos & 63) == 0;
+            unsigned long long cand0 = 0;
+            bool cand_beyond = false;
+            if (rect_cull_now) {
+                const int bsub = qpos >> 6;
+                const int bx0 = (tile_col << C.item_w_log2) + bsub * C.sub_dx, br0 = (tile_row << C.tile_h_log2) + bsub * C.sub_dy;
+                const int bx1 = bx0 + C.tile_w - 1, by0 = row_to_y(C, br0), by1 = row_to_y(C, br0 + (64 >> C.tile_w_log2) - 1);
+                cand0 = __ballot(rect_overlaps(rect0, bx0, bx1, by0, by1));
+                for (int j0 = 64; j0 < C.bvh_leaf_count && !cand_beyond; j0 += 64)
+                    cand_beyond = __any(j0 + lane_r < C.bvh_leaf_count && rect_overlaps(C.leaf_rects[j0 + lane_r], bx0, bx1, by0, by1));
+            }
+            const bool no_cand = rect_cull_now && cand0 == 0 && !cand_beyond;
             if ((st & (ST_PHASE | ST_PIXEL)) == (PH_DONE | ST_PIXEL)) {
                 store_mine(C);
                 st &= ~ST_PIXEL;
@@ -1036,21 +1071,26 @@
                     if (px < C.width && prow < C.local_rows) {
                         in_frame = true;
                         pidx = static_cast<uint32_t>(prow) * static_cast<uint32_t>(C.width) + static_cast<uint32_t>(px);
-                        ray = make_ray(C, px, row_to_y(C, prow));
-                        rd = ray.d;
                         counters = 0;
-                        t = 0.0;
-                        st = PH_MARCH | ST_PIXEL;
-                        if (ACCEL == 2) {
-                            ri = make_ray_inv(ray);
-                            inv0 = ri.inv[0];
-                            inv1 = ri.inv[1];
-                            inv2 = ri.inv[2];
-                            st |= ((ri.par[0] ? 1 : 0) | (ri.par[1] ? 2 : 0) | (ri.par[2] ? 4 : 0)) << ST_PAR_SHIFT;
+                        if (no_cand) {
+                            t = RM_MAX_DIST;
+                            st = PH_DONE | ST_PIXEL;
+                        } else {
+                            ray = make_ray(C, px, row_to_y(C, prow));
+                            rd = ray.d;
+                            t = 0.0;
+                            st = PH_MARCH | ST_PIXEL;
+                            if (ACCEL == 2) {
+                                ri = make_ray_inv(ray);
+                                inv0 = ri.inv[0];
+                                inv1 = ri.inv[1];
+                                inv2 = ri.inv[2];
+                                st |= ((ri.par[0] ? 1 : 0) | (ri.par[1] ? 2 : 0) | (ri.par[2] ? 4 : 0)) << ST_PAR_SHIFT;
+                            }
                         }
                     }
                 }
-                if (ACCEL == 2) {
+                if (ACCEL == 2 && !no_cand) {
 #ifdef RM_STAMPS
                     const unsigned long long t_pr0 = __builtin_amdgcn_s_memtime();
 #endif
@@ -1063,9 +1103,9 @@
                     if (whole_batch) {
                         const int x0 = (tile_col << C.item_w_log2) + batch_sub * C.sub_dx;
                         const int r0 = (tile_row << C.tile_h_log2) + batch_sub * C.sub_dy;
-                        const Bundle B = make_bundle(C, x0, x0 + Q.tile_w - 1, row_to_y(C, r0),
-                                                     row_to_y(C, r0 + (64 >> C.tile_w_log2) - 1));
-                        hc = bvh_prologue_cull<REL>(scene_view<ACCEL, LDS, REL>(C, smem), C, B, in_frame, ray, ri, L, cur, lane_now());
+                        hc = bvh_prologue_cull<REL>(scene_view<ACCEL, LDS, REL>(C, smem), C, x0, x0 + Q.tile_w - 1, row_to_y(C, r0),
+                                                    row_to_y(C, r0 + (64 >> C.tile_w_log2) - 1), rect_cull_now, cand0, in_frame, ray,
+                                                    ri, L, cur, lane_now());
                     } else if (in_frame) {
                         RM_CNT(15)
                         hc = bvh_prologue<REL>(scene_view<ACCEL, LDS, REL>(C, smem), ray, ri, L, cur);
@@ -1588,6 +1628,9 @@
     const bool lds = plan.lds, rel = plan.rel;
     p.list_cap = plan.list_cap;
     p.step_box = plan.step_box;
+    if (p.accel != 2 || !p.leaf_rects || !p.bvh_leaves || p.bvh_leaf_count <= 0 || p.bvh_leaf_count > RM_RECT_CULL_MAX_LEAVES ||
+        p.width > 65536 || p.height > 65536)
+        p.rect_cull = 0;
     const size_t list_bytes = plan.list_bytes, scene_bytes = plan.scene_bytes, rel_bytes = static_cast<size_t>(p.bvh_nodes) * 48;
     size_t shmem = (lds ? scene_bytes : 0) + (rel ? rel_bytes + 16 : 0) + list_bytes + 16;
     if (p.lds_fill && p.blocks_per_cu >= 2 && p.blocks_per_cu <= 8) {
@@ -1610,6 +1653,7 @@
         shape[1] = 256;
         shape[2] = static_cast<uint32_t>(shmem);
         shape[3] = p.step_box ? 1u : 0u;
+        shape[4] = p.rect_cull ? 1u : 0u;
     }
     hipError_t e = hipSuccess;
     if (!p.diag_block) e = hipMemsetAsync(p.tile_counters, 0, RM_QUEUES * RM_QSTRIDE * sizeof(unsigned int), stream);
diff --git a/cpu_raymarcher_amd/csrc/rm_rtc.cpp b/cpu_raymarcher_amd/csrc/rm_rtc.cpp
--- a/cpu_raymarcher_amd/csrc/rm_rtc.cpp
+++ b/cpu_raymarcher_amd/csrc/rm_rtc.cpp
@@ -464,6 +464,7 @@
     const char *render_fn;
     const char *distance_fn;
     std::string display;
+    bool no_machine_licm;
     bool no_scratch;
 };
 
@@ -506,6 +507,10 @@
     }
     std::vector<const char *> opts = {"--offload-arch=gfx950", "-O3", "-std=c++17", "-ffp-contract=off", "-fno-fast-math", "-mllvm", "-amdgpu-inline-max-bb=100000"};
     opts.push_back("-Rpass-analysis=kernel-resource-usage");
+    if (u.no_machine_licm) {
+        opts.push_back("-mllvm");
+        opts.push_back("-disable-machine-licm");
+    }
     const auto t0 = std::chrono::steady_clock::now();
     const hiprtcResult res = r.compile(prog, static_cast<int>(opts.size()), opts.data());
     out.compile_seconds = std::chrono::duration<double>(std::chrono::steady_clock::now() - t0).count();
@@ -581,6 +586,7 @@
     u.distance_fn = "rm_rtc_distance";
     u.display = std::string("rm_rtc_render<") + std::to_string(accel) + ", " + (other ? "true" : "false") + ">" + (length_sqrt ? " [length=sqrt]" : "");
     u.no_scratch = false;
+    u.no_machine_licm = false;
     return compile_unit(u, load_module, out, log);
 }
 
@@ -616,7 +622,8 @@
     return h;
 }
 
-bool compile_v2(const std::string &fixed_src, int accel, bool lds, bool ur, bool rel, bool length_sqrt, bool load_module, Kernel &out, std::string &log) {
+bool compile_v2(const std::string &fixed_src, int accel, bool lds, bool ur, bool rel, bool length_sqrt, bool no_machine_licm, bool load_module, Kernel &out,
+                std::string &log) {
     Unit u;
     u.defines = "#define RM_RTC_V2 1\n#define RM_RTC_V2_ACCEL " + std::to_string(accel) + "\n#define RM_RTC_V2_LDS " + (lds ? "1" : "0") + "\n#define RM_RTC_V2_UR " +
                 (ur ? "1" : "0") + "\n#define RM_RTC_V2_REL " + (rel ? "1" : "0") + "\n" + (length_sqrt ? "#define RM_LENGTH_SQRT 1\n" : "");
@@ -627,6 +634,7 @@
     u.distance_fn = nullptr;
     u.display = "rm_rtc_render_v2";
     u.no_scratch = true;
+    u.no_machine_licm = no_machine_licm;
     return compile_unit(u, load_module, out, log);
 }
 
@@ -646,7 +654,7 @@
     return std::to_string(device) + "|" + std::to_string(accel) + (other ? "|o" : "|s") + (length_sqrt ? "|q|" : "|h|") + (env ? env : "") + "|" + scene_src;
 }
 bool compile_any(const std::string &src, int accel, bool other, bool length_sqrt, Kernel &out, std::string &log) {
-    if (accel & kV2Bit) return compile_v2(src, accel & 3, (accel >> 2) & 1, (accel >> 3) & 1, (accel >> 4) & 1, length_sqrt, true, out, log);
+    if (accel & kV2Bit) return compile_v2(src, accel & 3, (accel >> 2) & 1, (accel >> 3) & 1, (accel >> 4) & 1, length_sqrt, (accel & kV2NoLicmBit) != 0, true, out, log);
     return compile(src, accel, other, length_sqrt, true, out, log);
 }
 int lookup(Cache &c, const std::string &key, Kernel &out, std::string &log) {
diff --git a/cpu_raymarcher_amd/csrc/rm_rtc.h b/cpu_raymarcher_amd/csrc/rm_rtc.h
--- a/cpu_raymarcher_amd/csrc/rm_rtc.h
+++ b/cpu_raymarcher_amd/csrc/rm_rtc.h
@@ -28,7 +28,9 @@
 
 std::string v2_fixed_source(const RmRenderParams &p, bool with_counts);
 uint64_t v2_fixed_hash(const RmRenderParams &p, int variant_bits);
-bool compile_v2(const std::string &fixed_src, int accel, bool lds, bool ur, bool rel, bool length_sqrt, bool load_module, Kernel &out, std::string &log);
+bool compile_v2(const std::string &fixed_src, int accel, bool lds, bool ur, bool rel, bool length_sqrt, bool no_machine_licm, bool load_module, Kernel &out,
+                std::string &log);
+constexpr int kV2NoLicmBit = 1 << 10;
 constexpr int kV2Bit = 1 << 8;
 
 constexpr int kCacheEntries = 256;
diff --git a/cpu_raymarcher_amd/csrc/rm_types.h b/cpu_raymarcher_amd/csrc/rm_types.h
--- a/cpu_raymarcher_amd/csrc/rm_types.h
+++ b/cpu_raymarcher_amd/csrc/rm_types.h
@@ -85,6 +85,11 @@
 };
 
 #define RM_V2_WAVES 6
+
+struct alignas(8) RmLeafRect {
+    uint16_t x_lo, x_hi, y_lo, y_hi;
+};
+#define RM_RECT_CULL_MAX_LEAVES 256
 
 struct RmRenderParams {
     int32_t width, height, y_start, y_end;
@@ -193,4 +198,6 @@
     float sb_origin[3], sb_inv[3];
     int32_t sb_bins, sb_stride;
     int32_t step_box;
-};
+    RmLeafRect *leaf_rects;
+    int32_t rect_cull;
+};
diff --git a/cpu_raymarcher_amd/csrc/rm_v2_fields.h b/cpu_raymarcher_amd/csrc/rm_v2_fields.h
--- a/cpu_raymarcher_amd/csrc/rm_v2_fields.h
+++ b/cpu_raymarcher_amd/csrc/rm_v2_fields.h
@@ -4,7 +4,7 @@
     X(width) X(height) X(accel) X(shader) X(tile_w) X(nodes_in_lds) X(filter) X(variant) X(list_cap) X(coop) X(use_grid)         \
     X(refill_threshold) X(hw_xcd) X(item_px) X(rel_boxes) X(lpt_stride) X(prim_filter) X(n0_batch) X(use_nn) X(tile_w_log2)     \
     X(tile_h_log2) X(tiles_x) X(item_wide) X(item_w_log2) X(sub_dx) X(sub_dy) X(tiles_x_magic) X(leaf_order) X(algorithm)       \
-    X(general) X(uniform_radius) X(multi_step) X(use_ext) X(step_box) X(sb_bins) X(sb_stride)
+    X(general) X(uniform_radius) X(multi_step) X(use_ext) X(step_box) X(sb_bins) X(sb_stride) X(rect_cull)
 
 #define RM_V2_FIXED_COUNTS(X)                                                                                                    \
     X(n_prims) X(bvh_nodes) X(oct_nodes) X(bvh_prim_count) X(oct_prim_count) X(pq_cell_count) X(pq_list_count) X(bvh_leaf_count) \
diff --git a/include/rm_raymarch.h b/include/rm_raymarch.h
--- a/include/rm_raymarch.h
+++ b/include/rm_raymarch.h
@@ -400,6 +400,9 @@
 RM_API int rm_debug_last_launch(rm_ctx *ctx, uint32_t out[4]);
 RM_API int rm_debug_overlap_fill(rm_ctx *ctx, int32_t asked, int64_t items, int32_t *effective);
 RM_API int rm_debug_step_box(rm_ctx *ctx, int32_t out[6]);
+RM_API int rm_debug_rect_cull(rm_ctx *ctx, const float *rot9, const float *origin3, int32_t width, int32_t height, int32_t out[5]);
+RM_API int rm_debug_leaf_rects(rm_ctx *ctx, const float *rot9, const float *origin3, int32_t width, int32_t height,
+                               uint16_t *rects, int32_t *nodes, int64_t cap, int64_t *n);
 RM_API int rm_debug_read_wave_times(rm_ctx *ctx, uint64_t *out24576);
 RM_API int rm_debug_read_batch_log(rm_ctx *ctx, uint32_t *out196608);
 
```
